# hbell99/DirectVoxGO

Measured on AMD Instinct MI355X. Metric: train rays/sec (8192-ray batch, 160^3 grid), higher is better.
Workload: dtype f32

## Files before the change

directvoxgo_amd/csrc/shade.hip:

```cpp
#include "common.h"
#include "x3.h"

#include <type_traits>


static int g_shade_experiment = 0;
static int g_shade_variant = 67;
extern "C" int dvgo_shade_wgrad_x3(const float* G1, const float* gz, const uint64_t* masks, const float* W3, const float* H1,
                                   const float* H2, const float* feat, int C, const float* emb, int E, const int64_t* ray_id,
                                   int64_t M, const int64_t* m_dev, int width, int diffuse, int n_parts, float* part, int form_b,
                                   void* stream);
extern "C" int dvgo_shade_bwd_x3(const float* g_rgb, const float* rgb, const uint64_t* masks, int64_t M, const int64_t* m_dev,
                                 const float* W1, const float* W2, const float* W3, int width, int d_in, int C, int diffuse,
                                 float* g_feat, float* G1, float* gz, void* scratch, int prebuilt, void* stream);

extern "C" int dvgo_shade_fwd_x3(const float* feat, int C, const float* emb, int E, const int64_t* ray_id, int64_t M, const int64_t* m_dev,
                                 const float* W1, const float* b1, const float* W2, const float* b2, const float* W3,
                                 const float* b3, int width, int d_in, int diffuse, float* rgb, float* H1, float* H2,
                                 uint64_t* masks, void* scratch, void* scratch_bwd, int experiment, void* stream);

#define SHADE_THREADS 768
#define SHADE_WAVES (SHADE_THREADS / 64)
#define SHADE_BWD_THREADS 1024
#define SHADE_BWD_WAVES (SHADE_BWD_THREADS / 64)

template <int WIDTH, int S1>
struct ShadeLds {
  static constexpr int T = WIDTH / 32;
  float w1a[T][S1][64];
  float w2a[T][T][16][64];
  float w3p[3][2][T * 16];
  float b1p[2][T * 16];
  float b2p[2][T * 16];
  float b3[4];
};

__device__ __forceinline__ int acc_feature(int t, int r, int h) { return 32 * t + (r & 3) + 8 * (r >> 2) + 4 * h; }

#define SHADE_STAGE_STRIDE 36
__device__ __forceinline__ void shade_store_tile(float* __restrict__ stage ,
                                                 const f32x16& acc, float* __restrict__ dst , int row_stride, int lane, int rows_valid) {
  const int smp = lane & 31, h = lane >> 5;
#pragma unroll
  for (int q = 0; q < 4; ++q)
    *reinterpret_cast<float4*>(stage + smp * SHADE_STAGE_STRIDE + 8 * q + 4 * h) =
        make_float4(acc[4 * q], acc[4 * q + 1], acc[4 * q + 2], acc[4 * q + 3]);
  const int c = lane & 7;
#pragma unroll
  for (int i = 0; i < 4; ++i) {
    const int r = (lane >> 3) + 8 * i;
    const float4 v = *reinterpret_cast<const float4*>(stage + r * SHADE_STAGE_STRIDE + 4 * c);
    if (r < rows_valid) *reinterpret_cast<float4*>(dst + (int64_t)r * row_stride + 4 * c) = v;
  }
}

template <int WIDTH, int S1>
__device__ __forceinline__ void shade_load_weights(ShadeLds<WIDTH, S1>& L, const float* __restrict__ W1,
                                                   const float* __restrict__ b1, const float* __restrict__ W2,
                                                   const float* __restrict__ b2, const float* __restrict__ W3,
                                                   const float* __restrict__ b3, int D_in) {
  constexpr int T = WIDTH / 32;
  const int tid = threadIdx.x, nt = blockDim.x;
  for (int i = tid; i < T * S1 * 64; i += nt) {
    const int l = i & 63, s = (i >> 6) % S1, t = (i >> 6) / S1;
    const int k = 2 * s + (l >> 5);
    (&L.w1a[0][0][0])[i] = (k < D_in) ? W1[(32 * t + (l & 31)) * D_in + k] : 0.0f;
  }
  for (int i = tid; i < T * T * 16 * 64; i += nt) {
    const int l = i & 63, r = (i >> 6) & 15, t = (i >> 10) % T, t2 = (i >> 10) / T;
    (&L.w2a[0][0][0][0])[i] = W2[(32 * t2 + (l & 31)) * WIDTH + acc_feature(t, r, l >> 5)];
  }
  for (int i = tid; i < 3 * 2 * T * 16; i += nt) {
    const int tr = i % (T * 16), h = (i / (T * 16)) & 1, c = i / (2 * T * 16);
    (&L.w3p[0][0][0])[i] = W3[c * WIDTH + acc_feature(tr >> 4, tr & 15, h)];
  }
  for (int i = tid; i < 2 * T * 16; i += nt) {
    const int tr = i % (T * 16), h = i / (T * 16);
    const int f = acc_feature(tr >> 4, tr & 15, h);
    (&L.b1p[0][0])[i] = b1[f];
    (&L.b2p[0][0])[i] = b2[f];
  }
  if (tid < 3) L.b3[tid] = b3[tid];
}

template <int WIDTH, int S1>
__device__ __forceinline__ void shade_tile_forward(const ShadeLds<WIDTH, S1>& L, const float (&x)[S1], int lane,
                                                   f32x16 (&acc1)[WIDTH / 32], float (&z)[3],
                                                   float* __restrict__ H2tile ,
                                                   float* __restrict__ stage, int rows_valid,
                                                   unsigned long long& mask2 ) {
  constexpr int T = WIDTH / 32;
  const int h = lane >> 5;
#pragma unroll
  for (int t = 0; t < T; ++t) {
#pragma unroll
    for (int r = 0; r < 16; ++r) acc1[t][r] = L.b1p[h][t * 16 + r];
#pragma unroll
    for (int s = 0; s < S1; ++s) acc1[t] = __builtin_amdgcn_mfma_f32_32x32x2f32(L.w1a[t][s][lane], x[s], acc1[t], 0, 0, 0);
#pragma unroll
    for (int r = 0; r < 16; ++r) acc1[t][r] = dvgo_relu(acc1[t][r]);
    __builtin_amdgcn_sched_barrier(0);
  }
  float p[3] = {0.0f, 0.0f, 0.0f};
  mask2 = 0ull;
#pragma unroll 1
  for (int t2 = 0; t2 < T; ++t2) {
    f32x16 acc2;
#pragma unroll
    for (int r = 0; r < 16; ++r) acc2[r] = L.b2p[h][t2 * 16 + r];
#pragma unroll
    for (int t = 0; t < T; ++t) {
#pragma unroll
      for (int r = 0; r < 16; ++r)
        acc2 = __builtin_amdgcn_mfma_f32_32x32x2f32(L.w2a[t2][t][r][lane], acc1[t][r], acc2, 0, 0, 0);
      __builtin_amdgcn_sched_barrier(0);
    }
#pragma unroll
    for (int r = 0; r < 16; ++r) acc2[r] = dvgo_relu(acc2[r]);
    if (H2tile != nullptr) {
      unsigned int bits = 0u;
#pragma unroll
      for (int r = 0; r < 16; ++r) bits |= dvgo_relu_bit(acc2[r]) << r;
      mask2 |= (unsigned long long)bits << (16 * t2);
      shade_store_tile(stage, acc2, H2tile + 32 * t2, WIDTH, lane, rows_valid);
    }
#pragma unroll
    for (int c = 0; c < 3; ++c) {
#pragma unroll
      for (int r = 0; r < 16; ++r) p[c] = fmaf(L.w3p[c][h][t2 * 16 + r], acc2[r], p[c]);
    }
  }
#pragma unroll
  for (int c = 0; c < 3; ++c) z[c] = p[c] + __shfl_xor(p[c], 32) + L.b3[c];
}

template <int S1>
__device__ __forceinline__ void shade_load_x(const float* __restrict__ feat, int C, int c_view0, int n_view,
                                             const float* __restrict__ emb, int E, int64_t row, int64_t ray,
                                             int lane, float (&x)[S1]) {
  const int h = lane >> 5;
  const float* fr = feat + row * C + c_view0;
  const float* er = emb + ray * E - n_view;
#pragma unroll
  for (int s = 0; s < S1; ++s) {
    const int k = 2 * s + h;
    float v = 0.0f;
    if (k < n_view) v = fr[k];
    else if (k < n_view + E) v = er[k];
    x[s] = v;
  }
}

template <int WIDTH, int S1, bool DIFFUSE>
__global__ void __launch_bounds__(SHADE_THREADS)
shade_fwd_kernel(const float* __restrict__ feat, int C, int c_view0, int n_view, const float* __restrict__ emb, int E,
                 const int64_t* __restrict__ ray_id, int64_t M_cap, const int64_t* __restrict__ m_dev, const float* __restrict__ W1,
                 const float* __restrict__ b1, const float* __restrict__ W2, const float* __restrict__ b2,
                 const float* __restrict__ W3, const float* __restrict__ b3, int D_in, float* __restrict__ rgb,
                 float* __restrict__ H1, float* __restrict__ H2, unsigned long long* __restrict__ masks, int experiment) {
  const int64_t M = m_dev ? (*m_dev < M_cap ? *m_dev : M_cap) : M_cap;
  constexpr int T = WIDTH / 32;
  __shared__ ShadeLds<WIDTH, S1> L;
  __shared__ __attribute__((aligned(16))) float s_stage[SHADE_WAVES][32 * SHADE_STAGE_STRIDE];
  shade_load_weights<WIDTH, S1>(L, W1, b1, W2, b2, W3, b3, D_in);
  __syncthreads();
  const int lane = threadIdx.x & 63, h = lane >> 5;
  float* stage = s_stage[threadIdx.x >> 6];
  const int64_t n_tiles = (M + 31) / 32;
  const int64_t gw = (int64_t)blockIdx.x * (blockDim.x >> 6) + (threadIdx.x >> 6);
  const int64_t nw = (int64_t)gridDim.x * (blockDim.x >> 6);
  for (int64_t tile = gw; tile < n_tiles; tile += nw) {
    const int64_t row = tile * 32 + (lane & 31);
    const bool valid = row < M;
    const int64_t rowc = valid ? row : (M - 1);
    float x[S1];
    if (experiment & 16) { for (int s = 0; s < S1; ++s) x[s] = 0.01f * (float)(lane + s); }
    else shade_load_x<S1>(feat, C, c_view0, n_view, emb, E, rowc, ray_id[rowc], lane, x);
    f32x16 acc1[T];
    float z[3];
    const int rows_valid = (int)(M - tile * 32 < 32 ? M - tile * 32 : 32);
    unsigned long long mask2;
    shade_tile_forward<WIDTH, S1>(L, x, lane, acc1, z, (H1 != nullptr && !(experiment & 32)) ? (H2 + tile * 32 * WIDTH) : nullptr,
                                  stage, rows_valid, mask2);
    if (valid) {
      if (h == 0) {
#pragma unroll
        for (int c = 0; c < 3; ++c) {
          const float zz = DIFFUSE ? z[c] + feat[row * C + c] : z[c];
          rgb[row * 3 + c] = 1.0f / (1.0f + expf(-zz));
        }
      }
      if (H1 != nullptr) {
        unsigned long long mask1 = 0ull;
#pragma unroll
        for (int t = 0; t < T; ++t) {
#pragma unroll
          for (int r = 0; r < 16; ++r) mask1 |= (unsigned long long)dvgo_relu_bit(acc1[t][r]) << (16 * t + r);
        }
        masks[(row * 2 + 0) * 2 + h] = mask1;
        masks[(row * 2 + 1) * 2 + h] = mask2;
      }
    }
    if (H1 != nullptr && !(experiment & 32)) {
#pragma unroll
      for (int t = 0; t < T; ++t) shade_store_tile(stage, acc1[t], H1 + tile * 32 * WIDTH + 32 * t, WIDTH, lane, rows_valid);
    }
  }
}

template <int WIDTH>
struct ShadeBwdLds {
  static constexpr int T = WIDTH / 32;
  float w2ta[T][T][16][64];
  float w1ta[T][16][64];
  float w3p[3][2][T * 16];
};

template <int WIDTH, bool DIFFUSE>
__global__ void __launch_bounds__(SHADE_BWD_THREADS)
shade_bwd_kernel(const float* __restrict__ g_rgb, const float* __restrict__ rgb,
                 const unsigned long long* __restrict__ masks, int64_t M_cap, const int64_t* __restrict__ m_dev,
                 const float* __restrict__ W1, const float* __restrict__ W2,
                 const float* __restrict__ W3, int D_in, int C, int c_view0, int n_view,
                 float* __restrict__ g_feat, float* __restrict__ G1, float* __restrict__ gz_out, int experiment) {
  const int64_t M = m_dev ? (*m_dev < M_cap ? *m_dev : M_cap) : M_cap;
  constexpr int T = WIDTH / 32;
  __shared__ ShadeBwdLds<WIDTH> L;
  __shared__ __attribute__((aligned(16))) float s_stage[SHADE_BWD_WAVES][32 * SHADE_STAGE_STRIDE];
  float* stage = s_stage[threadIdx.x >> 6];
  {
    const int tid = threadIdx.x, nt = blockDim.x;
    for (int i = tid; i < T * T * 16 * 64; i += nt) {
      const int l = i & 63, r = (i >> 6) & 15, t2 = (i >> 10) % T, tin = (i >> 10) / T;
      (&L.w2ta[0][0][0][0])[i] = W2[acc_feature(t2, r, l >> 5) * WIDTH + 32 * tin + (l & 31)];
    }
    for (int i = tid; i < T * 16 * 64; i += nt) {
      const int l = i & 63, r = (i >> 6) & 15, t = i >> 10;
      const int k = l & 31;
      (&L.w1ta[0][0][0])[i] = (k < D_in) ? W1[acc_feature(t, r, l >> 5) * D_in + k] : 0.0f;
    }
    for (int i = tid; i < 3 * 2 * T * 16; i += nt) {
      const int tr = i % (T * 16), h = (i / (T * 16)) & 1, c = i / (2 * T * 16);
      (&L.w3p[0][0][0])[i] = W3[c * WIDTH + acc_feature(tr >> 4, tr & 15, h)];
    }
  }
  __syncthreads();
  const int lane = threadIdx.x & 63, h = lane >> 5;
  const int64_t n_tiles = (M + 31) / 32;
  const int64_t gw = (int64_t)blockIdx.x * (blockDim.x >> 6) + (threadIdx.x >> 6);
  const int64_t nw = (int64_t)gridDim.x * (blockDim.x >> 6);
  for (int64_t tile = gw; tile < n_tiles; tile += nw) {
    const int64_t row = tile * 32 + (lane & 31);
    const bool valid = row < M;
    const int64_t rowc = valid ? row : (M - 1);
    float gz[3];
#pragma unroll
    for (int c = 0; c < 3; ++c) {
      const float o = rgb[rowc * 3 + c];
      gz[c] = valid ? g_rgb[rowc * 3 + c] * o * (1.0f - o) : 0.0f;
    }
    if (valid && h == 0) {
#pragma unroll
      for (int c = 0; c < 3; ++c) {
        gz_out[row * 3 + c] = gz[c];
        if (DIFFUSE) g_feat[row * C + c] = gz[c];
      }
    }
    const unsigned long long m1 = masks[(rowc * 2 + 0) * 2 + h];
    const unsigned long long m2 = masks[(rowc * 2 + 1) * 2 + h];
    f32x16 g2[T];
#pragma unroll
    for (int t2 = 0; t2 < T; ++t2) {
#pragma unroll
      for (int r = 0; r < 16; ++r) {
        const float v = fmaf(L.w3p[2][h][t2 * 16 + r], gz[2],
                             fmaf(L.w3p[1][h][t2 * 16 + r], gz[1], L.w3p[0][h][t2 * 16 + r] * gz[0]));
        g2[t2][r] = ((m2 >> (16 * t2 + r)) & 1ull) ? v : 0.0f;
      }
    }
    f32x16 gx;
#pragma unroll
    for (int r = 0; r < 16; ++r) gx[r] = 0.0f;
#pragma unroll 1
    for (int tin = 0; tin < T; ++tin) {
      f32x16 acc;
#pragma unroll
      for (int r = 0; r < 16; ++r) acc[r] = 0.0f;
#pragma unroll
      for (int t2 = 0; t2 < T; ++t2) {
#pragma unroll
        for (int r = 0; r < 16; ++r)
          acc = __builtin_amdgcn_mfma_f32_32x32x2f32(L.w2ta[tin][t2][r][lane], g2[t2][r], acc, 0, 0, 0);
        __builtin_amdgcn_sched_barrier(0);
      }
#pragma unroll
      for (int q = 0; q < 4; ++q) {
        const unsigned int mb = (unsigned int)(m1 >> (16 * tin + 4 * q)) & 15u;
        acc[4 * q + 0] = (mb & 1u) ? acc[4 * q + 0] : 0.0f;
        acc[4 * q + 1] = (mb & 2u) ? acc[4 * q + 1] : 0.0f;
        acc[4 * q + 2] = (mb & 4u) ? acc[4 * q + 2] : 0.0f;
        acc[4 * q + 3] = (mb & 8u) ? acc[4 * q + 3] : 0.0f;
      }
      if (!(experiment & 1))
        shade_store_tile(stage, acc, G1 + tile * 32 * WIDTH + 32 * tin, WIDTH, lane,
                         (int)(M - tile * 32 < 32 ? M - tile * 32 : 32));
#pragma unroll
      for (int r = 0; r < 16; ++r)
        gx = __builtin_amdgcn_mfma_f32_32x32x2f32(L.w1ta[tin][r][lane], acc[r], gx, 0, 0, 0);
    }
    if (valid) {
#pragma unroll
      for (int r = 0; r < 16; ++r) {
        const int k = (r & 3) + 8 * (r >> 2) + 4 * h;
        if (k < n_view) g_feat[row * C + c_view0 + k] = gx[r];
      }
    }
  }
}

template <int WIDTH>
struct ShadeWgradLds {
  float g1[1][32][WIDTH], h1[1][32][WIDTH], h2[1][32][WIDTH];
  float x[1][32][40];
  float gz[1][32][4];
  unsigned int m2[1][32][2][2];
};

typedef const __attribute__((address_space(1))) void* dvgo_gptr_t;
typedef __attribute__((address_space(3))) void* dvgo_lptr_t;

template <int WIDTH>
__global__ void __launch_bounds__(2 * WIDTH) __attribute__((amdgpu_num_vgpr(104)))
shade_wgrad_kernel(const float* __restrict__ G1, const float* __restrict__ gz, const unsigned int* __restrict__ masks,
                   const float* __restrict__ W3, const float* __restrict__ H1, const float* __restrict__ H2, const float* __restrict__ feat, int C,
                   int c_view0, int n_view, const float* __restrict__ emb, int E, const int64_t* __restrict__ ray_id,
                   int64_t M_cap, const int64_t* __restrict__ m_dev,
                   float* __restrict__ part ) {
  const int64_t M = m_dev ? (*m_dev < M_cap ? *m_dev : M_cap) : M_cap;
  constexpr int T = WIDTH / 32;
  static_assert(T == 4 || T == 2, "widths 128 and 64");
  constexpr int TPR = 2 * T;
  constexpr int NXI = 40 / TPR;
  constexpr int LPR = WIDTH / 4;
  constexpr int RPI = 64 / LPR;
  __shared__ __attribute__((aligned(16))) ShadeWgradLds<WIDTH> L;
  const int tid = threadIdx.x, lane = tid & 63, h = lane >> 5, j = lane & 31, w = tid >> 6;
  f32x16 aW2[T], aW1;
  float vW3[3] = {0.0f, 0.0f, 0.0f};
  float vW1[8];
#pragma unroll
  for (int t = 0; t < T; ++t)
#pragma unroll
    for (int r = 0; r < 16; ++r) aW2[t][r] = 0.0f;
#pragma unroll
  for (int r = 0; r < 16; ++r) aW1[r] = 0.0f;
#pragma unroll
  for (int kk = 0; kk < 8; ++kk) vW1[kk] = 0.0f;
  float sb1 = 0.0f, sb2 = 0.0f, gz_acc = 0.0f;
  const float w30 = W3[32 * w + j], w31 = W3[WIDTH + 32 * w + j], w32 = W3[2 * WIDTH + 32 * w + j];
  const int m_half = (j >> 2) & 1, m_word = w >> 1, m_bit = 16 * (w & 1) + (j & 3) + 4 * (j >> 3);
  const int d_in = n_view + E;
  const int64_t n_tiles = (M + 31) / 32;

  float px[NXI], pgz;
  unsigned int pm2;
  bool pvalid, pgvalid;
  int64_t ray_nx;
  const int xrow = tid / TPR, xcol = tid - xrow * TPR;
  {
    const int64_t row = (int64_t)blockIdx.x * 32 + xrow;
    ray_nx = M > 0 ? ray_id[row < M ? row : M - 1] : 0;
  }
#define SHADE_WGRAD_DMA(TILE, BUF)                                                                              \
  {                                                                                                             \
    const int64_t r0_ = (TILE) * 32;                                                                            \
    {                                                                                                           \
      const int64_t row = r0_ + xrow;                                                                           \
      const int64_t rc = row < M ? row : M - 1;                                                                 \
      const float* fr = feat + rc * C + c_view0;                                                                \
      const float* er = emb + ray_nx * E - n_view;                     \
      _Pragma("unroll") for (int i = 0; i < NXI; ++i) {                          \
        const int k = xcol + TPR * i;                                                                           \
        const int kc = k < d_in ? k : d_in - 1;                                                                 \
        px[i] = *((kc < n_view) ? fr + kc : er + kc);                                                           \
      }                                                                                                         \
      pvalid = row < M;                                                                                         \
      const int64_t row2 = r0_ + (int64_t)gridDim.x * 32 + xrow;                                                \
      ray_nx = ray_id[row2 < M ? row2 : M - 1];                        \
    }                                                                                                           \
    {                                                                                                           \
      const int64_t row = r0_ + ((tid & 127) >> 2);                                                             \
      const int64_t rc = row < M ? row : M - 1;                                                                 \
      pgz = gz[rc * 3 + ((tid & 3) < 3 ? (tid & 3) : 0)];                                                       \
      pgvalid = (tid & 3) < 3 && row < M;                                                                       \
       \
      pm2 = masks[rc * 8 + 4 + (tid & 3)];                                                                      \
    }                                                                                                           \
                           \
    _Pragma("unroll") for (int i = 0; i < 4; ++i) {             \
      const int rl = (4 * w + i) * RPI;                  \
      const int64_t row = r0_ + rl + lane / LPR;                                                                \
      const int64_t off = (row < M ? row : M - 1) * WIDTH + 4 * (lane % LPR);                                   \
      __builtin_amdgcn_global_load_lds((dvgo_gptr_t)(G1 + off), (dvgo_lptr_t)&L.g1[BUF][rl][0], 16, 0, 0);     \
      __builtin_amdgcn_global_load_lds((dvgo_gptr_t)(H1 + off), (dvgo_lptr_t)&L.h1[BUF][rl][0], 16, 0, 0);     \
      __builtin_amdgcn_global_load_lds((dvgo_gptr_t)(H2 + off), (dvgo_lptr_t)&L.h2[BUF][rl][0], 16, 0, 0);     \
    }                                                                                                           \
  }

  constexpr int buf = 0;
  for (int64_t tile = blockIdx.x; tile < n_tiles; tile += gridDim.x) {
    SHADE_WGRAD_DMA(tile, 0);
    asm volatile("" : "+v"(px[0]), "+v"(px[1]), "+v"(px[2]), "+v"(px[3]), "+v"(px[4]), "+v"(pgz), "+v"(pm2));
    if (NXI > 5) asm volatile("" : "+v"(px[NXI - 5]), "+v"(px[NXI - 4]), "+v"(px[NXI - 3]), "+v"(px[NXI - 2]), "+v"(px[NXI - 1]));
#pragma unroll
    for (int i = 0; i < NXI; ++i) L.x[buf][xrow][xcol + TPR * i] = (pvalid && xcol + TPR * i < d_in) ? px[i] : 0.0f;
    if (tid < 128) {
      gz_acc += pgvalid ? pgz : 0.0f;
      L.gz[buf][tid >> 2][tid & 3] = pgvalid ? pgz : 0.0f;
      (&L.m2[buf][tid >> 2][0][0])[tid & 3] = pm2;
    }
    __builtin_amdgcn_s_waitcnt(0x0F70);
    __syncthreads();
    const int rows_valid = (int)(M - tile * 32 < 32 ? M - tile * 32 : 32);
#pragma unroll 4
    for (int s = 0; s < 16; ++s) {
      const int row = 2 * s + h;
      const float4 gzr = *reinterpret_cast<const float4*>(&L.gz[buf][row][0]);
      const float g2v = fmaf(w32, gzr.z, fmaf(w31, gzr.y, w30 * gzr.x));
      const float a2 = ((L.m2[buf][row][m_half][m_word] >> m_bit) & 1u) ? g2v : 0.0f;
      const float a1 = row < rows_valid ? L.g1[buf][row][32 * w + j] : 0.0f;
      sb2 += a2; sb1 += a1;
#pragma unroll
      for (int t = 0; t < T; ++t)
        aW2[t] = __builtin_amdgcn_mfma_f32_32x32x2f32(a2, L.h1[buf][row][32 * t + j], aW2[t], 0, 0, 0);
      aW1 = __builtin_amdgcn_mfma_f32_32x32x2f32(a1, L.x[buf][row][j], aW1, 0, 0, 0);
      const float4 xa = *reinterpret_cast<const float4*>(&L.x[buf][row][32]);
      const float4 xb = *reinterpret_cast<const float4*>(&L.x[buf][row][36]);
      vW1[0] = fmaf(a1, xa.x, vW1[0]); vW1[1] = fmaf(a1, xa.y, vW1[1]); vW1[2] = fmaf(a1, xa.z, vW1[2]);
      vW1[3] = fmaf(a1, xa.w, vW1[3]); vW1[4] = fmaf(a1, xb.x, vW1[4]); vW1[5] = fmaf(a1, xb.y, vW1[5]);
      vW1[6] = fmaf(a1, xb.z, vW1[6]); vW1[7] = fmaf(a1, xb.w, vW1[7]);
      const float hv = L.h2[buf][row][32 * w + j];
      vW3[0] = fmaf(gzr.x, hv, vW3[0]); vW3[1] = fmaf(gzr.y, hv, vW3[1]); vW3[2] = fmaf(gzr.z, hv, vW3[2]);
    }
    __syncthreads();
  }
#undef SHADE_WGRAD_DMA
  float* p = part + (int64_t)blockIdx.x * (WIDTH * WIDTH + WIDTH * 64 + 32 * WIDTH + 3 * WIDTH);
  float* pW2 = p;
  float* pW1 = pW2 + WIDTH * WIDTH;
  float* pW3 = pW1 + WIDTH * 64;
  float* pb = pW3 + 32 * WIDTH;
#pragma unroll
  for (int r = 0; r < 16; ++r) {
    const int i = (r & 3) + 8 * (r >> 2) + 4 * h;
#pragma unroll
    for (int t = 0; t < T; ++t) pW2[(32 * w + i) * WIDTH + 32 * t + j] = aW2[t][r];
    pW1[(32 * w + i) * 64 + j] = aW1[r];
  }
#pragma unroll
  for (int kk = 0; kk < 8; ++kk) {
    const float v = vW1[kk] + __shfl_xor(vW1[kk], 32);
    if (h == 0) pW1[(32 * w + j) * 64 + 32 + kk] = v;
  }
  if (h == 0) {
#pragma unroll
    for (int kk = 8; kk < 32; ++kk) pW1[(32 * w + j) * 64 + 32 + kk] = 0.0f;
  }
#pragma unroll
  for (int c = 0; c < 3; ++c) {
    const float v = vW3[c] + __shfl_xor(vW3[c], 32);
    if (h == 0) pW3[c * WIDTH + 32 * w + j] = v;
  }
  float gz_sum = gz_acc;
  gz_sum += __shfl_xor(gz_sum, 4); gz_sum += __shfl_xor(gz_sum, 8);
  gz_sum += __shfl_xor(gz_sum, 16); gz_sum += __shfl_xor(gz_sum, 32);
  sb1 += __shfl_xor(sb1, 32); sb2 += __shfl_xor(sb2, 32);
  if (h == 0) {
    pb[32 * w + j] = sb1;
    pb[WIDTH + 32 * w + j] = sb2;
    if (j < 8) pb[2 * WIDTH + 8 * w + j] = (w < 2 && j < 3) ? gz_sum : 0.0f;
    if (T == 2 && j >= 16) pb[2 * WIDTH + 16 * w + j] = 0.0f;
  }
}

__device__ __forceinline__ unsigned lds_addr(const void* p) {
  return (unsigned)(uintptr_t)(const __attribute__((address_space(3))) void*)p;
}
template <int OFF> __device__ __forceinline__ float lds_f32(unsigned a) {
  float v; asm volatile("ds_read_b32 %0, %1 offset:%2" : "=v"(v) : "v"(a), "n"(OFF)); return v;
}
template <int OFF> __device__ __forceinline__ unsigned lds_u32(unsigned a) {
  unsigned v; asm volatile("ds_read_b32 %0, %1 offset:%2" : "=v"(v) : "v"(a), "n"(OFF)); return v;
}
typedef float dvgo_f32x4 __attribute__((ext_vector_type(4)));
template <int OFF> __device__ __forceinline__ dvgo_f32x4 lds_f32x4(unsigned a) {
  dvgo_f32x4 v; asm volatile("ds_read_b128 %0, %1 offset:%2" : "=v"(v) : "v"(a), "n"(OFF)); return v;
}
template <int I, int N, typename F> __device__ __forceinline__ void static_for(F&& f) {
  if constexpr (I < N) { f(std::integral_constant<int, I>{}); static_for<I + 1, N>(f); }
}

template <int WIDTH>
struct ShadeWgradRing {
  static constexpr int NB = 2, NR = 4, TR = 16;
  float g1[NB][TR][WIDTH], h1[NB][TR][WIDTH], h2[NB][TR][WIDTH];
  float xf[NB][TR][16];
  float xe[NB][TR][32];
  float gz[NB][TR][4];
  unsigned int m2[NB][TR][4];
  unsigned int rid[NR][64];
};

template <int T>
struct WgradOperands {
  dvgo_f32x4 gq, xa, xb;
  unsigned mw;
  float g1v, h1v[T], xv, h2v;
};

#define DVGO_OOB 0x80000000u

template <int WIDTH>
__global__ void __launch_bounds__(2 * WIDTH, 2)
shade_wgrad_ring_kernel(const float* __restrict__ G1, const float* __restrict__ gz, const unsigned int* __restrict__ masks,
                        const float* __restrict__ W3, const float* __restrict__ H1, const float* __restrict__ H2,
                        const float* __restrict__ feat, int C, int c_view0, int n_view, const float* __restrict__ emb, int E,
                        const int64_t* __restrict__ ray_id, int64_t M_cap, const int64_t* __restrict__ m_dev,
                        float* __restrict__ part ,
                        float* __restrict__ total, int total_size ) {
#if defined(__HIP_DEVICE_COMPILE__)
  for (int i = blockIdx.x * blockDim.x + threadIdx.x; i < total_size; i += gridDim.x * blockDim.x) total[i] = 0.0f;
  int64_t M;
  {
    const int64_t m = m_dev ? (*m_dev < M_cap ? *m_dev : M_cap) : M_cap;
    M = ((int64_t)__builtin_amdgcn_readfirstlane((int)(m >> 32)) << 32) | (unsigned)__builtin_amdgcn_readfirstlane((int)m);
  }
  using Ring = ShadeWgradRing<WIDTH>;
  constexpr int T = WIDTH / 32, NW = T, NB = Ring::NB, NR = Ring::NR, TR = Ring::TR;
  static_assert(T == 4 || T == 2, "widths 128 and 64");
  constexpr int LPR = WIDTH / 4;
  constexpr int RPI = 64 / LPR;
  constexpr int IPW = TR / RPI / NW;
  constexpr int FPW = 4 / NW, EPW = 8 / NW;
  static_assert(IPW == 2 && NB == 2, "double buffer: the wait at the top of a tile is vmcnt(0)");
  __shared__ __attribute__((aligned(16))) Ring L;
  const int tid = threadIdx.x, lane = tid & 63, h = lane >> 5, j = lane & 31;
  const int w = __builtin_amdgcn_readfirstlane(tid >> 6);
  f32x16 aW2[T], aW1;
  float vW3[3] = {0.0f, 0.0f, 0.0f}, vW1[8], sgz[3] = {0.0f, 0.0f, 0.0f};
#pragma unroll
  for (int t = 0; t < T; ++t)
#pragma unroll
    for (int r = 0; r < 16; ++r) aW2[t][r] = 0.0f;
#pragma unroll
  for (int r = 0; r < 16; ++r) aW1[r] = 0.0f;
#pragma unroll
  for (int kk = 0; kk < 8; ++kk) vW1[kk] = 0.0f;
  float sb1 = 0.0f, sb2 = 0.0f;
  const float w30 = W3[32 * w + j], w31 = W3[WIDTH + 32 * w + j], w32 = W3[2 * WIDTH + 32 * w + j];
  const int m_idx = 2 * ((j >> 2) & 1) + (w >> 1), m_bit = 16 * (w & 1) + (j & 3) + 4 * (j >> 3);
  const int d_in = n_view + E;
  const int n_tiles = (int)((M + TR - 1) / TR);
  auto tile_of = [&](int k) { return (int)blockIdx.x + k * (int)gridDim.x; };

  const unsigned rows_b = (unsigned)(M * WIDTH * 4);
  const auto bG1 = __builtin_amdgcn_make_buffer_rsrc((void*)G1, 0, rows_b, 0x00020000);
  const auto bH1 = __builtin_amdgcn_make_buffer_rsrc((void*)H1, 0, rows_b, 0x00020000);
  const auto bH2 = __builtin_amdgcn_make_buffer_rsrc((void*)H2, 0, rows_b, 0x00020000);
  const auto bF = __builtin_amdgcn_make_buffer_rsrc((void*)feat, 0, (unsigned)(M * C * 4), 0x00020000);
  const auto bE = __builtin_amdgcn_make_buffer_rsrc((void*)emb, 0, DVGO_OOB, 0x00020000);
  const auto bGz = __builtin_amdgcn_make_buffer_rsrc((void*)gz, 0, (unsigned)(M * 12), 0x00020000);
  const auto bM = __builtin_amdgcn_make_buffer_rsrc((void*)masks, 0, (unsigned)(M * 32), 0x00020000);
  const auto bR = __builtin_amdgcn_make_buffer_rsrc((void*)ray_id, 0, (unsigned)(M * 8), 0x00020000);
  unsigned vo_bulk[IPW], vo_f[FPW], vo_ecol[EPW];
  int e_row[EPW];
#pragma unroll
  for (int i = 0; i < IPW; ++i) vo_bulk[i] = (unsigned)(((IPW * w + i) * RPI + lane / LPR) * WIDTH * 4 + 16 * (lane % LPR));
#pragma unroll
  for (int i = 0; i < FPW; ++i) {
    const int e = 64 * (w + NW * i) + lane, row = e >> 4, col = e & 15;
    vo_f[i] = col < n_view ? (unsigned)((row * C + c_view0 + col) * 4) : DVGO_OOB;
  }
#pragma unroll
  for (int i = 0; i < EPW; ++i) {
    const int e = 64 * (w + NW * i) + lane, col = e & 31;
    e_row[i] = e >> 5;
    vo_ecol[i] = col < E ? (unsigned)(col * 4) : DVGO_OOB;
  }
  const unsigned vo_gz = (lane & 3) < 3 ? (unsigned)(((lane >> 2) * 3 + (lane & 3)) * 4) : DVGO_OOB;
  const unsigned vo_m2 = (unsigned)(((lane >> 2) * 8 + 4 + (lane & 3)) * 4);
  const unsigned vo_rid = (unsigned)((lane & (TR - 1)) * 8);

  auto issue = [&](int t) {
    const int sl = t & (NB - 1);
    const unsigned r0 = (unsigned)__builtin_amdgcn_readfirstlane(tile_of(t) * TR);
#pragma unroll
    for (int i = 0; i < IPW; ++i) {
      const int rl = (IPW * w + i) * RPI;
      __builtin_amdgcn_raw_ptr_buffer_load_lds(bG1, (dvgo_lptr_t)&L.g1[sl][rl][0], 16, vo_bulk[i], r0 * (WIDTH * 4), 0, 0);
      __builtin_amdgcn_raw_ptr_buffer_load_lds(bH1, (dvgo_lptr_t)&L.h1[sl][rl][0], 16, vo_bulk[i], r0 * (WIDTH * 4), 0, 0);
      __builtin_amdgcn_raw_ptr_buffer_load_lds(bH2, (dvgo_lptr_t)&L.h2[sl][rl][0], 16, vo_bulk[i], r0 * (WIDTH * 4), 0, 0);
    }
#pragma unroll
    for (int i = 0; i < FPW; ++i)
      __builtin_amdgcn_raw_ptr_buffer_load_lds(bF, (dvgo_lptr_t)(&L.xf[sl][0][0] + 64 * (w + NW * i)), 4, vo_f[i], r0 * (unsigned)(C * 4), 0, 0);
    unsigned rids[EPW];
#pragma unroll
    for (int i = 0; i < EPW; ++i) rids[i] = lds_u32<0>(lds_addr(&L.rid[t & (NR - 1)][e_row[i]]));
    if constexpr (EPW == 2) asm volatile("s_waitcnt lgkmcnt(0)" : "+v"(rids[0]), "+v"(rids[1]));
    else asm volatile("s_waitcnt lgkmcnt(0)" : "+v"(rids[0]), "+v"(rids[1]), "+v"(rids[EPW - 2]), "+v"(rids[EPW - 1]));
#pragma unroll
    for (int i = 0; i < EPW; ++i)
      __builtin_amdgcn_raw_ptr_buffer_load_lds(bE, (dvgo_lptr_t)(&L.xe[sl][0][0] + 64 * (w + NW * i)), 4,
                                               vo_ecol[i] + rids[i] * (unsigned)(E * 4), 0, 0, 0);
    const unsigned rn = (unsigned)__builtin_amdgcn_readfirstlane(tile_of(t + 2) * TR);
    const int rsl = (t + 2) & (NR - 1);
    auto small = [&](int which) {
      if (which == 0) __builtin_amdgcn_raw_ptr_buffer_load_lds(bGz, (dvgo_lptr_t)&L.gz[sl][0][0], 4, vo_gz, r0 * 12u, 0, 0);
      else if (which == 1) __builtin_amdgcn_raw_ptr_buffer_load_lds(bM, (dvgo_lptr_t)&L.m2[sl][0][0], 4, vo_m2, r0 * 32u, 0, 0);
      else __builtin_amdgcn_raw_ptr_buffer_load_lds(bR, (dvgo_lptr_t)&L.rid[rsl][0], 4, vo_rid, rn * 8u, 0, 0);
    };
    if constexpr (NW == 4) {
      small(w < 2 ? w : 2);
    } else {
      small(w);
      small(2);
    }
  };

  const unsigned a_gz = lds_addr(&L.gz[0][h][0]), a_mw = lds_addr(&L.m2[0][h][m_idx]);
  const unsigned a_g1 = lds_addr(&L.g1[0][h][32 * w + j]), a_h1 = lds_addr(&L.h1[0][h][j]);
  const unsigned a_h2 = lds_addr(&L.h2[0][h][32 * w + j]);
  const bool x_in_f = j < n_view;
  const unsigned a_x = x_in_f ? lds_addr(&L.xf[0][h][j]) : lds_addr(&L.xe[0][h][j - n_view]);
  const unsigned x_slot = x_in_f ? (unsigned)(TR * 16 * 4) : (unsigned)(TR * 32 * 4), x_step = x_in_f ? 128u : 256u;
  const bool trail = d_in > 32;
  const unsigned a_xa = lds_addr(&L.xe[0][h][trail ? 32 - n_view : 0]);
  constexpr unsigned SLOT_ROWS = TR * WIDTH * 4;
  using Ops = WgradOperands<T>;
  auto wait_ops = [&](Ops& o) {
    if constexpr (T == 4)
      asm volatile("s_waitcnt lgkmcnt(0)" : "+v"(o.gq), "+v"(o.xa), "+v"(o.xb), "+v"(o.mw), "+v"(o.g1v), "+v"(o.h1v[0]),
                   "+v"(o.h1v[1]), "+v"(o.h1v[2]), "+v"(o.h1v[3]), "+v"(o.xv), "+v"(o.h2v));
    else
      asm volatile("s_waitcnt lgkmcnt(0)" : "+v"(o.gq), "+v"(o.xa), "+v"(o.xb), "+v"(o.mw), "+v"(o.g1v), "+v"(o.h1v[0]),
                   "+v"(o.h1v[1]), "+v"(o.xv), "+v"(o.h2v));
  };

  if (tid < 64) {
#pragma unroll
    for (int t = 0; t < 2; ++t) {
      const int64_t row = (int64_t)tile_of(t) * TR + (tid & (TR - 1));
      L.rid[t][tid] = row < M ? (unsigned int)ray_id[row] : 0u;
    }
  }
  __syncthreads();
#pragma unroll
  for (int t = 0; t < NB - 1; ++t) issue(t);
  for (int k = 0; tile_of(k) < n_tiles; ++k) {
    const int sl = k & (NB - 1);
    asm volatile("s_waitcnt vmcnt(0)\n\ts_waitcnt lgkmcnt(0)\n\ts_barrier" ::: "memory");
    issue(k + NB - 1);
    const unsigned b_gz = a_gz + sl * (TR * 16), b_mw = a_mw + sl * (TR * 16), b_g1 = a_g1 + sl * SLOT_ROWS;
    const unsigned b_h1 = a_h1 + sl * SLOT_ROWS, b_h2 = a_h2 + sl * SLOT_ROWS;
    const unsigned b_xa = a_xa + sl * (TR * 32 * 4);
    unsigned b_x = a_x + sl * x_slot;
    Ops ops[2];
    float a2s[2], a1s[2];
    auto read_ops = [&](auto Sc, Ops& o) {
      constexpr int s = decltype(Sc)::value;
      o.gq = lds_f32x4<32 * s>(b_gz);
      o.mw = lds_u32<32 * s>(b_mw);
      o.g1v = lds_f32<8 * WIDTH * s>(b_g1);
      static_for<0, T>([&](auto Tc) { constexpr int t = decltype(Tc)::value; o.h1v[t] = lds_f32<8 * WIDTH * s + 128 * t>(b_h1); });
      o.xv = lds_f32<0>(b_x);
      b_x += x_step;
      o.xa = lds_f32x4<256 * s>(b_xa);
      o.xb = lds_f32x4<256 * s + 16>(b_xa);
      o.h2v = lds_f32<8 * WIDTH * s>(b_h2);
    };
    auto prep = [&](const Ops& o, float& a2, float& a1) {
      const float g2v = fmaf(w32, o.gq.z, fmaf(w31, o.gq.y, w30 * o.gq.x));
      a2 = ((o.mw >> m_bit) & 1u) ? g2v : 0.0f;
      a1 = o.g1v;
    };
    read_ops(std::integral_constant<int, 0>{}, ops[0]);
    wait_ops(ops[0]);
    prep(ops[0], a2s[0], a1s[0]);
    static_for<0, TR / 2>([&](auto Sc) {
      constexpr int s = decltype(Sc)::value;
      constexpr bool more = s + 1 < TR / 2;
      Ops& cur = ops[s & 1];
      Ops& nxt = ops[(s + 1) & 1];
      const float a2 = a2s[s & 1], a1 = a1s[s & 1];
      aW2[0] = __builtin_amdgcn_mfma_f32_32x32x2f32(a2, cur.h1v[0], aW2[0], 0, 0, 0);
      if constexpr (more) read_ops(std::integral_constant<int, s + 1>{}, nxt);
      sb2 += a2; sb1 += a1;
      sgz[0] += cur.gq.x; sgz[1] += cur.gq.y; sgz[2] += cur.gq.z;
      __builtin_amdgcn_sched_barrier(0);
      aW2[1] = __builtin_amdgcn_mfma_f32_32x32x2f32(a2, cur.h1v[1], aW2[1], 0, 0, 0);
      vW1[0] = fmaf(a1, cur.xa.x, vW1[0]); vW1[1] = fmaf(a1, cur.xa.y, vW1[1]); vW1[2] = fmaf(a1, cur.xa.z, vW1[2]);
      vW1[3] = fmaf(a1, cur.xa.w, vW1[3]);
      vW3[0] = fmaf(cur.gq.x, cur.h2v, vW3[0]); vW3[1] = fmaf(cur.gq.y, cur.h2v, vW3[1]); vW3[2] = fmaf(cur.gq.z, cur.h2v, vW3[2]);
      __builtin_amdgcn_sched_barrier(0);
      if constexpr (T == 4) aW2[2] = __builtin_amdgcn_mfma_f32_32x32x2f32(a2, cur.h1v[2], aW2[2], 0, 0, 0);
      vW1[4] = fmaf(a1, cur.xb.x, vW1[4]); vW1[5] = fmaf(a1, cur.xb.y, vW1[5]); vW1[6] = fmaf(a1, cur.xb.z, vW1[6]);
      vW1[7] = fmaf(a1, cur.xb.w, vW1[7]);
      if constexpr (more) wait_ops(nxt);
      __builtin_amdgcn_sched_barrier(0);
      if constexpr (T == 4) aW2[3] = __builtin_amdgcn_mfma_f32_32x32x2f32(a2, cur.h1v[3], aW2[3], 0, 0, 0);
      if constexpr (more) prep(nxt, a2s[(s + 1) & 1], a1s[(s + 1) & 1]);
      __builtin_amdgcn_sched_barrier(0);
      aW1 = __builtin_amdgcn_mfma_f32_32x32x2f32(a1, cur.xv, aW1, 0, 0, 0);
      __builtin_amdgcn_sched_barrier(0);
    });
  }
  asm volatile("s_waitcnt vmcnt(0)" ::: "memory");
  float* p = part + (int64_t)blockIdx.x * (WIDTH * WIDTH + WIDTH * 64 + 32 * WIDTH + 3 * WIDTH);
  float* pW2 = p;
  float* pW1 = pW2 + WIDTH * WIDTH;
  float* pW3 = pW1 + WIDTH * 64;
  float* pb = pW3 + 32 * WIDTH;
#pragma unroll
  for (int r = 0; r < 16; ++r) {
    const int i = (r & 3) + 8 * (r >> 2) + 4 * h;
#pragma unroll
    for (int t = 0; t < T; ++t) pW2[(32 * w + i) * WIDTH + 32 * t + j] = aW2[t][r];
    pW1[(32 * w + i) * 64 + j] = aW1[r];
  }
#pragma unroll
  for (int kk = 0; kk < 8; ++kk) {
    const float v = vW1[kk] + __shfl_xor(vW1[kk], 32);
    if (h == 0) pW1[(32 * w + j) * 64 + 32 + kk] = (trail && 32 + kk < d_in) ? v : 0.0f;
  }
  if (h == 0) {
#pragma unroll
    for (int kk = 8; kk < 32; ++kk) pW1[(32 * w + j) * 64 + 32 + kk] = 0.0f;
  }
#pragma unroll
  for (int c = 0; c < 3; ++c) {
    const float v = vW3[c] + __shfl_xor(vW3[c], 32);
    if (h == 0) pW3[c * WIDTH + 32 * w + j] = v;
    sgz[c] += __shfl_xor(sgz[c], 32);
  }
  sb1 += __shfl_xor(sb1, 32); sb2 += __shfl_xor(sb2, 32);
  if (h == 0) {
    pb[32 * w + j] = sb1;
    pb[WIDTH + 32 * w + j] = sb2;
    if (j < 8) pb[2 * WIDTH + 8 * w + j] = (w == 0 && j < 3) ? sgz[j] : 0.0f;
    if (T == 2 && j >= 16) pb[2 * WIDTH + 16 * w + j] = 0.0f;
  }
#endif
}
typedef float dvgo_f32x2 __attribute__((ext_vector_type(2)));
template <int O0, int O1> __device__ __forceinline__ dvgo_f32x2 lds_f32_pair_st64(unsigned a) {
  dvgo_f32x2 v; asm volatile("ds_read2st64_b32 %0, %1 offset0:%2 offset1:%3" : "=v"(v) : "v"(a), "n"(O0), "n"(O1)); return v;
}
template <int O0, int O1> __device__ __forceinline__ dvgo_f32x2 lds_f32_pair(unsigned a) {
  dvgo_f32x2 v; asm volatile("ds_read2_b32 %0, %1 offset0:%2 offset1:%3" : "=v"(v) : "v"(a), "n"(O0), "n"(O1)); return v;
}
template <int OFF> __device__ __forceinline__ u32x4 lds_u32x4(unsigned a) {
  u32x4 v; asm volatile("ds_read_b128 %0, %1 offset:%2" : "=v"(v) : "v"(a), "n"(OFF)); return v;
}
template <int OFF> __device__ __forceinline__ void lds_store_u32x4(unsigned a, u32x4 v) {
  asm volatile("ds_write_b128 %0, %1 offset:%2" :: "v"(a), "v"(v), "n"(OFF) : "memory");
}

template <int WIDTH>
struct ShadeWgradRingX3 : ShadeWgradRing<WIDTH> {
  u32x4 fb[WIDTH / 32 + 2][3][64];
};

template <int WIDTH>
__global__ void __launch_bounds__(2 * WIDTH, 2)
shade_wgrad_ring_x3_kernel(const float* __restrict__ G1, const float* __restrict__ gz, const unsigned int* __restrict__ masks,
                           const float* __restrict__ W3, const float* __restrict__ H1, const float* __restrict__ H2,
                           const float* __restrict__ feat, int C, int c_view0, int n_view, const float* __restrict__ emb, int E,
                           const int64_t* __restrict__ ray_id, int64_t M_cap, const int64_t* __restrict__ m_dev,
                           float* __restrict__ part, float* __restrict__ total, int total_size) {
#if defined(__HIP_DEVICE_COMPILE__)
  for (int i = blockIdx.x * blockDim.x + threadIdx.x; i < total_size; i += gridDim.x * blockDim.x) total[i] = 0.0f;
  int64_t M;
  {
    const int64_t m = m_dev ? (*m_dev < M_cap ? *m_dev : M_cap) : M_cap;
    M = ((int64_t)__builtin_amdgcn_readfirstlane((int)(m >> 32)) << 32) | (unsigned)__builtin_amdgcn_readfirstlane((int)m);
  }
  using Ring = ShadeWgradRingX3<WIDTH>;
  constexpr int T = WIDTH / 32, NW = T, NB = Ring::NB, NR = Ring::NR, TR = Ring::TR;
  static_assert(T == 4 || T == 2, "widths 128 and 64");
  constexpr int LPR = WIDTH / 4, RPI = 64 / LPR, IPW = TR / RPI / NW;
  constexpr int DW = NW == 4 ? 2 : NW, FPW = 4 / DW, EPW = 8 / DW;
  static_assert(IPW == 2 && NB == 2 && TR == 16, "double buffer of 16-row tiles: the wait at the top of a tile is vmcnt(0)");
  __shared__ __attribute__((aligned(16))) Ring L;
  const int tid = threadIdx.x, lane = tid & 63, h = lane >> 5, j = lane & 31;
  const int w = __builtin_amdgcn_readfirstlane(tid >> 6);
  const int dw = NW == 4 ? w - 2 : w;
  f32x16 aW2[T], aW1[2];
  float vW3[3] = {0.0f, 0.0f, 0.0f}, sgz[3] = {0.0f, 0.0f, 0.0f};
#pragma unroll
  for (int t = 0; t < T; ++t)
#pragma unroll
    for (int r = 0; r < 16; ++r) aW2[t][r] = 0.0f;
#pragma unroll
  for (int q = 0; q < 2; ++q)
#pragma unroll
    for (int r = 0; r < 16; ++r) aW1[q][r] = 0.0f;
  float sb1 = 0.0f, sb2 = 0.0f;
  const float w30 = W3[32 * w + j], w31 = W3[WIDTH + 32 * w + j], w32 = W3[2 * WIDTH + 32 * w + j];
  const int m_idx = 2 * ((j >> 2) & 1) + (w >> 1);
  const unsigned m_bit = 16 * (w & 1) + (j & 3) + 4 * (j >> 3);
  const int d_in = n_view + E;
  const int n_tiles = (int)((M + TR - 1) / TR);
  auto tile_of = [&](int k) { return (int)blockIdx.x + k * (int)gridDim.x; };
  const unsigned rows_b = (unsigned)(M * WIDTH * 4);
  const auto bG1 = __builtin_amdgcn_make_buffer_rsrc((void*)G1, 0, rows_b, 0x00020000);
  const auto bH1 = __builtin_amdgcn_make_buffer_rsrc((void*)H1, 0, rows_b, 0x00020000);
  const auto bH2 = __builtin_amdgcn_make_buffer_rsrc((void*)H2, 0, rows_b, 0x00020000);
  const auto bF = __builtin_amdgcn_make_buffer_rsrc((void*)feat, 0, (unsigned)(M * C * 4), 0x00020000);
  const auto bE = __builtin_amdgcn_make_buffer_rsrc((void*)emb, 0, DVGO_OOB, 0x00020000);
  const auto bGz = __builtin_amdgcn_make_buffer_rsrc((void*)gz, 0, (unsigned)(M * 12), 0x00020000);
  const auto bM = __builtin_amdgcn_make_buffer_rsrc((void*)masks, 0, (unsigned)(M * 32), 0x00020000);
  const auto bR = __builtin_amdgcn_make_buffer_rsrc((void*)ray_id, 0, (unsigned)(M * 8), 0x00020000);
  unsigned vo_bulk[IPW], vo_f[FPW], vo_ecol[EPW];
  int e_row[EPW];
#pragma unroll
  for (int i = 0; i < IPW; ++i) vo_bulk[i] = (unsigned)(((IPW * w + i) * RPI + lane / LPR) * WIDTH * 4 + 16 * (lane % LPR));
#pragma unroll
  for (int i = 0; i < FPW; ++i) {
    const int e = 64 * ((dw < 0 ? 0 : dw) + DW * i) + lane, row = e >> 4, col = e & 15;
    vo_f[i] = col < n_view ? (unsigned)((row * C + c_view0 + col) * 4) : DVGO_OOB;
  }
#pragma unroll
  for (int i = 0; i < EPW; ++i) {
    const int e = 64 * ((dw < 0 ? 0 : dw) + DW * i) + lane, col = e & 31;
    e_row[i] = e >> 5;
    vo_ecol[i] = col < E ? (unsigned)(col * 4) : DVGO_OOB;
  }
  const unsigned vo_gz = (lane & 3) < 3 ? (unsigned)(((lane >> 2) * 3 + (lane & 3)) * 4) : DVGO_OOB;
  const unsigned vo_m2 = (unsigned)(((lane >> 2) * 8 + 4 + (lane & 3)) * 4);
  const unsigned vo_rid = (unsigned)((lane & (TR - 1)) * 8);
  auto issue = [&](int t) {
    const int sl = t & (NB - 1);
    const unsigned r0 = (unsigned)__builtin_amdgcn_readfirstlane(tile_of(t) * TR);
#pragma unroll
    for (int i = 0; i < IPW; ++i) {
      const int rl = (IPW * w + i) * RPI;
      __builtin_amdgcn_raw_ptr_buffer_load_lds(bG1, (dvgo_lptr_t)&L.g1[sl][rl][0], 16, vo_bulk[i], r0 * (WIDTH * 4), 0, 0);
      __builtin_amdgcn_raw_ptr_buffer_load_lds(bH1, (dvgo_lptr_t)&L.h1[sl][rl][0], 16, vo_bulk[i], r0 * (WIDTH * 4), 0, 0);
      __builtin_amdgcn_raw_ptr_buffer_load_lds(bH2, (dvgo_lptr_t)&L.h2[sl][rl][0], 16, vo_bulk[i], r0 * (WIDTH * 4), 0, 0);
    }
    if (dw < 0) return;
#pragma unroll
    for (int i = 0; i < FPW; ++i)
      __builtin_amdgcn_raw_ptr_buffer_load_lds(bF, (dvgo_lptr_t)(&L.xf[sl][0][0] + 64 * (dw + DW * i)), 4, vo_f[i], r0 * (unsigned)(C * 4), 0, 0);
    unsigned rids[EPW];
#pragma unroll
    for (int i = 0; i < EPW; ++i) rids[i] = lds_u32<0>(lds_addr(&L.rid[t & (NR - 1)][e_row[i]]));
    asm volatile("s_waitcnt lgkmcnt(0)" : "+v"(rids[0]), "+v"(rids[1]), "+v"(rids[2]), "+v"(rids[3]));
#pragma unroll
    for (int i = 0; i < EPW; ++i)
      __builtin_amdgcn_raw_ptr_buffer_load_lds(bE, (dvgo_lptr_t)(&L.xe[sl][0][0] + 64 * (dw + DW * i)), 4,
                                               vo_ecol[i] + rids[i] * (unsigned)(E * 4), 0, 0, 0);
    const unsigned rn = (unsigned)__builtin_amdgcn_readfirstlane(tile_of(t + 2) * TR);
    const int rsl = (t + 2) & (NR - 1);
    auto small = [&](int which) {
      if (which == 0) __builtin_amdgcn_raw_ptr_buffer_load_lds(bGz, (dvgo_lptr_t)&L.gz[sl][0][0], 4, vo_gz, r0 * 12u, 0, 0);
      else if (which == 1) __builtin_amdgcn_raw_ptr_buffer_load_lds(bM, (dvgo_lptr_t)&L.m2[sl][0][0], 4, vo_m2, r0 * 32u, 0, 0);
      else __builtin_amdgcn_raw_ptr_buffer_load_lds(bR, (dvgo_lptr_t)&L.rid[rsl][0], 4, vo_rid, rn * 8u, 0, 0);
    };
    if (dw == 0) { small(0); small(1); } else small(2);
  };
  const unsigned a_gz = lds_addr(&L.gz[0][8 * h][0]), a_mw = lds_addr(&L.m2[0][8 * h][m_idx]);
  const unsigned a_g1 = lds_addr(&L.g1[0][8 * h][32 * w + j]), a_h1 = lds_addr(&L.h1[0][8 * h][32 * w + j]);
  const unsigned a_h2 = lds_addr(&L.h2[0][8 * h][32 * w + j]);
  const int xcol = 32 * (w & 1) + j;
  const bool x_in_f = xcol < n_view, x_ok = xcol < d_in;
  const unsigned a_x = x_in_f ? lds_addr(&L.xf[0][8 * h][xcol]) : lds_addr(&L.xe[0][8 * h][x_ok ? xcol - n_view : 0]);
  const unsigned a_fb = lds_addr(&L.fb[0][0][lane]);
  constexpr unsigned SLOT_ROWS = TR * WIDTH * 4, FB_TILE = 3 * 64 * 16, FB_PIECE = 64 * 16;
  if (tid < 64) {
#pragma unroll
    for (int t = 0; t < 2; ++t) {
      const int64_t row = (int64_t)tile_of(t) * TR + (tid & (TR - 1));
      L.rid[t][tid] = row < M ? (unsigned int)ray_id[row] : 0u;
    }
  }
  __syncthreads();
#pragma unroll
  for (int t = 0; t < NB - 1; ++t) issue(t);
  for (int k = 0; tile_of(k) < n_tiles; ++k) {
    const int sl = k & (NB - 1);
    asm volatile("s_waitcnt vmcnt(0)\n\ts_waitcnt lgkmcnt(0)\n\ts_barrier" ::: "memory");
    issue(k + NB - 1);
    const unsigned b_gz = a_gz + sl * (TR * 16), b_mw = a_mw + sl * (TR * 16), b_g1 = a_g1 + sl * SLOT_ROWS;
    const unsigned b_h1 = a_h1 + sl * SLOT_ROWS, b_h2 = a_h2 + sl * SLOT_ROWS;
    const unsigned b_x = a_x + sl * (x_in_f ? (unsigned)(TR * 16 * 4) : (unsigned)(TR * 32 * 4));
    dvgo_f32x4 gq[8];
    unsigned mw[8];
    float g1v[8], h1v[8], h2v[8], xv[8];
    constexpr int RS = WIDTH * 4 / 256;
    static_for<0, 4>([&](auto Ec) {
      constexpr int e = 2 * decltype(Ec)::value;
      const dvgo_f32x2 v = lds_f32_pair_st64<e * RS, (e + 1) * RS>(b_h1);
      h1v[e] = v.x; h1v[e + 1] = v.y;
    });
    if (w < 2) {
      if (x_in_f) static_for<0, 8>([&](auto Ec) { constexpr int e = decltype(Ec)::value; xv[e] = lds_f32<e * 16 * 4>(b_x); });
      else static_for<0, 8>([&](auto Ec) { constexpr int e = decltype(Ec)::value; xv[e] = lds_f32<e * 32 * 4>(b_x); });
    }
    static_for<0, 8>([&](auto Ec) {
      constexpr int e = decltype(Ec)::value;
      gq[e] = lds_f32x4<16 * e>(b_gz);
    });
    static_for<0, 4>([&](auto Ec) {
      constexpr int e = 2 * decltype(Ec)::value;
      const dvgo_f32x2 m = lds_f32_pair<4 * e, 4 * (e + 1)>(b_mw);
      mw[e] = __float_as_uint(m.x); mw[e + 1] = __float_as_uint(m.y);
      const dvgo_f32x2 a = lds_f32_pair_st64<e * RS, (e + 1) * RS>(b_g1);
      g1v[e] = a.x; g1v[e + 1] = a.y;
      const dvgo_f32x2 b = lds_f32_pair_st64<e * RS, (e + 1) * RS>(b_h2);
      h2v[e] = b.x; h2v[e + 1] = b.y;
    });
    asm volatile("s_waitcnt lgkmcnt(0)" : "+v"(h1v[0]), "+v"(h1v[1]), "+v"(h1v[2]), "+v"(h1v[3]), "+v"(h1v[4]), "+v"(h1v[5]),
                 "+v"(h1v[6]), "+v"(h1v[7]), "+v"(gq[0]), "+v"(gq[1]), "+v"(gq[2]), "+v"(gq[3]), "+v"(gq[4]), "+v"(gq[5]), "+v"(gq[6]),
                 "+v"(gq[7]));
    asm volatile("" : "+v"(mw[0]), "+v"(mw[1]), "+v"(mw[2]), "+v"(mw[3]), "+v"(mw[4]), "+v"(mw[5]), "+v"(mw[6]), "+v"(mw[7]),
                 "+v"(g1v[0]), "+v"(g1v[1]), "+v"(g1v[2]), "+v"(g1v[3]), "+v"(g1v[4]), "+v"(g1v[5]), "+v"(g1v[6]), "+v"(g1v[7]));
    asm volatile("" : "+v"(h2v[0]), "+v"(h2v[1]), "+v"(h2v[2]), "+v"(h2v[3]), "+v"(h2v[4]), "+v"(h2v[5]), "+v"(h2v[6]), "+v"(h2v[7]));
    {
      u32x4 p0, p1, p2;
      x3_split8(h1v, p0, p1, p2);
      lds_store_u32x4<0>(a_fb + w * FB_TILE, p0);
      lds_store_u32x4<FB_PIECE>(a_fb + w * FB_TILE, p1);
      lds_store_u32x4<2 * FB_PIECE>(a_fb + w * FB_TILE, p2);
      if (w < 2) {
        asm volatile("" : "+v"(xv[0]), "+v"(xv[1]), "+v"(xv[2]), "+v"(xv[3]), "+v"(xv[4]), "+v"(xv[5]), "+v"(xv[6]), "+v"(xv[7]));
#pragma unroll
        for (int e = 0; e < 8; ++e) xv[e] = x_ok ? xv[e] : 0.0f;
        x3_split8(xv, p0, p1, p2);
        lds_store_u32x4<0>(a_fb + (T + w) * FB_TILE, p0);
        lds_store_u32x4<FB_PIECE>(a_fb + (T + w) * FB_TILE, p1);
        lds_store_u32x4<2 * FB_PIECE>(a_fb + (T + w) * FB_TILE, p2);
      }
    }
    u32x4 a2f[3], a1f[3];
    {
      float a2[8];
#pragma unroll
      for (int e = 0; e < 8; ++e) {
        const float g2v = fmaf(w32, gq[e].z, fmaf(w31, gq[e].y, w30 * gq[e].x));
        a2[e] = __uint_as_float(__float_as_uint(g2v) & (unsigned)__builtin_amdgcn_sbfe((int)mw[e], m_bit, 1u));
        sb2 += a2[e]; sb1 += g1v[e];
        vW3[0] = fmaf(gq[e].x, h2v[e], vW3[0]); vW3[1] = fmaf(gq[e].y, h2v[e], vW3[1]); vW3[2] = fmaf(gq[e].z, h2v[e], vW3[2]);
      }
      if (w == 0) {
#pragma unroll
        for (int e = 0; e < 8; ++e) { sgz[0] += gq[e].x; sgz[1] += gq[e].y; sgz[2] += gq[e].z; }
      }
      x3_split8(a2, a2f[0], a2f[1], a2f[2]);
      x3_split8(g1v, a1f[0], a1f[1], a1f[2]);
    }
    asm volatile("s_waitcnt lgkmcnt(0)\n\ts_barrier" ::: "memory");
    u32x4 fr[2][2][3];
    auto read_pair = [&](auto Pc, u32x4 (&f)[2][3]) {
      constexpr int p = decltype(Pc)::value;
#pragma unroll
      for (int q = 0; q < 3; ++q) {
        f[0][q] = lds_u32x4<(2 * p) * FB_TILE>(a_fb + q * FB_PIECE);
        f[1][q] = lds_u32x4<(2 * p + 1) * FB_TILE>(a_fb + q * FB_PIECE);
      }
    };
    auto wait_pair = [&](u32x4 (&f)[2][3]) {
      asm volatile("s_waitcnt lgkmcnt(0)" : "+v"(f[0][0]), "+v"(f[0][1]), "+v"(f[0][2]), "+v"(f[1][0]), "+v"(f[1][1]), "+v"(f[1][2]));
    };
    auto mfma_pair = [&](f32x16& accA, f32x16& accB, const u32x4 (&a)[3], const u32x4 (&f)[2][3]) {
#define X3D_MF(ACC, A, B) ACC = __builtin_amdgcn_mfma_f32_32x32x16_bf16(__builtin_bit_cast(bf16x8, A), __builtin_bit_cast(bf16x8, B), ACC, 0, 0, 0)
      X3D_MF(accA, a[2], f[0][0]); X3D_MF(accB, a[2], f[1][0]);
      X3D_MF(accA, a[1], f[0][1]); X3D_MF(accB, a[1], f[1][1]);
      X3D_MF(accA, a[0], f[0][2]); X3D_MF(accB, a[0], f[1][2]);
      X3D_MF(accA, a[1], f[0][0]); X3D_MF(accB, a[1], f[1][0]);
      X3D_MF(accA, a[0], f[0][1]); X3D_MF(accB, a[0], f[1][1]);
      X3D_MF(accA, a[0], f[0][0]); X3D_MF(accB, a[0], f[1][0]);
#undef X3D_MF
    };
    constexpr int NP = T / 2 + 1;
    read_pair(std::integral_constant<int, 0>{}, fr[0]);
    static_for<0, NP>([&](auto Pc) {
      constexpr int p = decltype(Pc)::value;
      wait_pair(fr[p & 1]);
      if constexpr (p + 1 < NP) read_pair(std::integral_constant<int, p + 1>{}, fr[(p + 1) & 1]);
      if constexpr (p < T / 2) mfma_pair(aW2[2 * p], aW2[2 * p + 1], a2f, fr[p & 1]);
      else mfma_pair(aW1[0], aW1[1], a1f, fr[p & 1]);
      __builtin_amdgcn_sched_barrier(0);
    });
  }
  asm volatile("s_waitcnt vmcnt(0)" ::: "memory");
  float* p = part + (int64_t)blockIdx.x * (WIDTH * WIDTH + WIDTH * 64 + 32 * WIDTH + 3 * WIDTH);
  float* pW2 = p;
  float* pW1 = pW2 + WIDTH * WIDTH;
  float* pW3 = pW1 + WIDTH * 64;
  float* pb = pW3 + 32 * WIDTH;
#pragma unroll
  for (int r = 0; r < 16; ++r) {
    const int i = (r & 3) + 8 * (r >> 2) + 4 * h;
#pragma unroll
    for (int t = 0; t < T; ++t) pW2[(32 * w + i) * WIDTH + 32 * t + j] = aW2[t][r];
    pW1[(32 * w + i) * 64 + j] = aW1[0][r];
    pW1[(32 * w + i) * 64 + 32 + j] = aW1[1][r];
  }
#pragma unroll
  for (int c = 0; c < 3; ++c) {
    const float v = vW3[c] + __shfl_xor(vW3[c], 32);
    if (h == 0) pW3[c * WIDTH + 32 * w + j] = v;
    sgz[c] += __shfl_xor(sgz[c], 32);
  }
  sb1 += __shfl_xor(sb1, 32); sb2 += __shfl_xor(sb2, 32);
  if (h == 0) {
    pb[32 * w + j] = sb1;
    pb[WIDTH + 32 * w + j] = sb2;
    if (j < 8) pb[2 * WIDTH + 8 * w + j] = (w == 0 && j < 3) ? sgz[j] : 0.0f;
    if (T == 2 && j >= 16) pb[2 * WIDTH + 16 * w + j] = 0.0f;
  }
#endif
}
#undef DVGO_OOB

#define SHADE_REDUCE_SLICES 16
__global__ void __launch_bounds__(256)
shade_wgrad_reduce_kernel(const float* __restrict__ part, int n_parts, int n, int W, int d_in, float* __restrict__ out) {
  const int i = blockIdx.x * blockDim.x + threadIdx.x;
  if (i >= n) return;
  int o;
  const int nW2 = W * W, nW1 = W * 64, nW3 = 32 * W;
  if (i < nW2) o = i;
  else if (i < nW2 + nW1) {
    const int r = (i - nW2) >> 6, c = (i - nW2) & 63;
    o = c < d_in ? nW2 + r * d_in + c : -1;
  } else if (i < nW2 + nW1 + nW3) {
    const int e = i - nW2 - nW1;
    o = e < 3 * W ? nW2 + W * d_in + e : -1;
  } else {
    const int e = i - nW2 - nW1 - nW3, base = nW2 + W * d_in + 3 * W;
    if (e < 2 * W) o = base + e;
    else {
      const int c = e - 2 * W;
      o = c < 3 ? base + 2 * W + c : (c >= 8 && c < 11) ? base + 2 * W + c - 8 : -1;
    }
  }
  if (o < 0) return;
  const int per = (n_parts + SHADE_REDUCE_SLICES - 1) / SHADE_REDUCE_SLICES;
  const int p0 = blockIdx.y * per, p1 = min(n_parts, p0 + per);
  float a0 = 0.0f, a1 = 0.0f, a2 = 0.0f, a3 = 0.0f;
  int p = p0;
  for (; p + 4 <= p1; p += 4) {
    a0 += part[(int64_t)p * n + i];
    a1 += part[(int64_t)(p + 1) * n + i];
    a2 += part[(int64_t)(p + 2) * n + i];
    a3 += part[(int64_t)(p + 3) * n + i];
  }
  for (; p < p1; ++p) a0 += part[(int64_t)p * n + i];
  if (p1 > p0) atomicAdd(out + o, (a0 + a1) + (a2 + a3));
}

extern "C" {

int dvgo_shade_fwd(const float* feat, int C, const float* emb, int E, const int64_t* ray_id, int64_t M, const int64_t* m_dev,
                   const float* W1, const float* b1, const float* W2, const float* b2, const float* W3,
                   const float* b3, int width, int d_in, int diffuse, float* rgb, float* H1, float* H2,
                   uint64_t* masks, void* scratch, void* scratch_bwd, void* stream) {
  if (M < 0 || C <= 0 || E < 0) return DVGO_EINVAL;
  if (M == 0) return 0;
  if (!feat || !emb || !ray_id || !W1 || !b1 || !W2 || !b2 || !W3 || !b3 || !rgb) return DVGO_EINVAL;
  if ((H1 == nullptr) != (H2 == nullptr) || (H1 == nullptr) != (masks == nullptr)) return DVGO_EINVAL;
  const int c_view0 = diffuse ? 3 : 0;
  const int n_view = C - c_view0;
  if (n_view < 0 || d_in != n_view + E) return DVGO_EINVAL;
  if ((width != 128 && width != 64) || d_in > 40) return DVGO_ERANGE;
  if ((g_shade_variant & 1) && scratch != nullptr)
    return dvgo_shade_fwd_x3(feat, C, emb, E, ray_id, M, m_dev, W1, b1, W2, b2, W3, b3, width, d_in, diffuse, rgb, H1, H2, masks,
                             scratch, (g_shade_variant & 2) ? scratch_bwd : nullptr, g_shade_experiment, stream);
  hipStream_t s = (hipStream_t)stream;
  const int64_t n_tiles = (M + 31) / 32;
  const int64_t cap = width == 128 ? 256 : 512;
  int blocks = (int)((n_tiles + SHADE_WAVES - 1) / SHADE_WAVES < cap ? (n_tiles + SHADE_WAVES - 1) / SHADE_WAVES : cap);
#define DVGO_SHADE(W, S1, DIFF)                                                                           \
  shade_fwd_kernel<W, S1, DIFF><<<blocks, SHADE_THREADS, 0, s>>>(feat, C, c_view0, n_view, emb, E, ray_id, M, m_dev, W1, b1, W2, \
                                                          b2, W3, b3, d_in, rgb, H1, H2, (unsigned long long*)masks, g_shade_experiment)
  if (width == 128) {
    if (d_in <= 36) { if (diffuse) DVGO_SHADE(128, 18, true); else DVGO_SHADE(128, 18, false); }
    else            { if (diffuse) DVGO_SHADE(128, 20, true); else DVGO_SHADE(128, 20, false); }
  } else {
    if (d_in <= 12) { if (diffuse) DVGO_SHADE(64, 6, true); else DVGO_SHADE(64, 6, false); }
    else            { if (diffuse) DVGO_SHADE(64, 20, true); else DVGO_SHADE(64, 20, false); }
  }
#undef DVGO_SHADE
  DVGO_LAUNCH_CHECK();
  return 0;
}

int dvgo_shade_experiment(int flags) { g_shade_experiment = flags; return 0; }

int dvgo_shade_variant(int flags) { const int old = g_shade_variant; if (flags >= 0) g_shade_variant = flags; return old; }

int dvgo_shade_bwd(const float* g_rgb, const float* rgb, const uint64_t* masks, int64_t M, const int64_t* m_dev,
                   const float* W1, const float* W2, const float* W3, int width, int d_in, int C, int diffuse,
                   float* g_feat, float* G1, float* gz, void* scratch, int prebuilt, void* stream) {
  if (M < 0 || C <= 0) return DVGO_EINVAL;
  if (M == 0) return 0;
  if (!g_rgb || !rgb || !masks || !W1 || !W2 || !W3 || !g_feat || !G1 || !gz) return DVGO_EINVAL;
  const int c_view0 = diffuse ? 3 : 0;
  const int n_view = C - c_view0;
  if ((width != 128 && width != 64) || n_view < 0 || n_view > 32 || d_in < n_view) return DVGO_ERANGE;
  if ((g_shade_variant & 2) && scratch != nullptr)
    return dvgo_shade_bwd_x3(g_rgb, rgb, masks, M, m_dev, W1, W2, W3, width, d_in, C, diffuse, g_feat, G1, gz, scratch, prebuilt, stream);
  hipStream_t s = (hipStream_t)stream;
  const int64_t n_tiles = (M + 31) / 32;
  const int64_t cap = width == 128 ? 256 : 512;
  int blocks = (int)((n_tiles + SHADE_BWD_WAVES - 1) / SHADE_BWD_WAVES < cap ? (n_tiles + SHADE_BWD_WAVES - 1) / SHADE_BWD_WAVES : cap);
#define DVGO_SHADE_BWD(W, DIFF)                                                                                                       \
  shade_bwd_kernel<W, DIFF><<<blocks, SHADE_BWD_THREADS, 0, s>>>(g_rgb, rgb, (const unsigned long long*)masks, M, m_dev, W1, W2, W3, d_in, C, c_view0, \
                                                            n_view, g_feat, G1, gz, g_shade_experiment)
  if (width == 128) { if (diffuse) DVGO_SHADE_BWD(128, true); else DVGO_SHADE_BWD(128, false); }
  else              { if (diffuse) DVGO_SHADE_BWD(64, true); else DVGO_SHADE_BWD(64, false); }
#undef DVGO_SHADE_BWD
  DVGO_LAUNCH_CHECK();
  return 0;
}

int dvgo_shade_wgrad(const float* G1, const float* gz, const uint64_t* masks, const float* W3, const float* H1,
                     const float* H2, const float* feat, int C, const float* emb, int E, const int64_t* ray_id, int64_t M,
                     const int64_t* m_dev, int width, int diffuse, int n_parts, float* part, float* total, void* stream) {
  if (M < 0 || n_parts <= 0 || C <= 0 || E < 0) return DVGO_EINVAL;
  if (!G1 || !gz || !masks || !W3 || !H1 || !H2 || !feat || !emb || !ray_id || !part || !total) return DVGO_EINVAL;
  const int c_view0 = diffuse ? 3 : 0;
  const int n_view = C - c_view0;
  if ((width != 128 && width != 64) || n_view < 0 || n_view + E > 40) return DVGO_ERANGE;
  bool ring = false;
  if (g_shade_variant & (4 | 32)) {
    const int form_b = (g_shade_variant & 32) ? 2 : (g_shade_variant & 16) ? 1 : 0;
    if (!form_b && n_parts > 256) n_parts = 256;
    const int rc = dvgo_shade_wgrad_x3(G1, gz, masks, W3, H1, H2, feat, C, emb, E, ray_id, M, m_dev, width, diffuse, n_parts, part,
                                       form_b, stream);
    if (rc != 0) return rc;
  } else if (!(g_shade_variant & 8) && n_view <= 16 && E <= 32 && (n_view + E <= 32 || (n_view % 4 == 0 && n_view >= 8)) &&
             M * width * 4 < ((int64_t)1 << 31) && M * C * 4 < ((int64_t)1 << 31)) {
    if (n_parts > 512) n_parts = 512;
    ring = true;
    const int tsz = width * width + width * (n_view + E) + 5 * width + 3;
    if ((g_shade_variant & 64) && width == 128)
      shade_wgrad_ring_x3_kernel<128><<<n_parts, 256, 0, (hipStream_t)stream>>>(
          G1, gz, (const unsigned int*)masks, W3, H1, H2, feat, C, c_view0, n_view, emb, E, ray_id, M, m_dev, part, total, tsz);
    else if (g_shade_variant & 64)
      shade_wgrad_ring_x3_kernel<64><<<n_parts, 128, 0, (hipStream_t)stream>>>(
          G1, gz, (const unsigned int*)masks, W3, H1, H2, feat, C, c_view0, n_view, emb, E, ray_id, M, m_dev, part, total, tsz);
    else if (width == 128)
      shade_wgrad_ring_kernel<128><<<n_parts, 256, 0, (hipStream_t)stream>>>(
          G1, gz, (const unsigned int*)masks, W3, H1, H2, feat, C, c_view0, n_view, emb, E, ray_id, M, m_dev, part, total, tsz);
    else
      shade_wgrad_ring_kernel<64><<<n_parts, 128, 0, (hipStream_t)stream>>>(
          G1, gz, (const unsigned int*)masks, W3, H1, H2, feat, C, c_view0, n_view, emb, E, ray_id, M, m_dev, part, total, tsz);
  } else if (width == 128)
    shade_wgrad_kernel<128><<<n_parts, 256, 0, (hipStream_t)stream>>>(
        G1, gz, (const unsigned int*)masks, W3, H1, H2, feat, C, c_view0, n_view, emb, E, ray_id, M, m_dev, part);
  else
    shade_wgrad_kernel<64><<<n_parts, 128, 0, (hipStream_t)stream>>>(
        G1, gz, (const unsigned int*)masks, W3, H1, H2, feat, C, c_view0, n_view, emb, E, ray_id, M, m_dev, part);
  DVGO_LAUNCH_CHECK();
  const int psize = width * width + width * 64 + 32 * width + 3 * width;
  const int d_in = n_view + E;
  const int tsize = width * width + width * d_in + 3 * width + 2 * width + 3;
  if (!ring && hipMemsetAsync(total, 0, (size_t)tsize * sizeof(float), (hipStream_t)stream) != hipSuccess) return DVGO_EINVAL;
  shade_wgrad_reduce_kernel<<<dim3((psize + 255) / 256, SHADE_REDUCE_SLICES), 256, 0, (hipStream_t)stream>>>(part, n_parts, psize,
                                                                                                       width, d_in, total);
  DVGO_LAUNCH_CHECK();
  return 0;
}

}
```

directvoxgo_amd/csrc/shade_x3.hip:

```cpp
#include "common.h"
#include "x3.h"

#ifndef X3_THREADS
#define X3_THREADS 512
#endif
#define X3_WAVES (X3_THREADS / 64)
#ifndef X3_BWD_THREADS
#define X3_BWD_THREADS 512
#endif
#define X3_BWD_WAVES (X3_BWD_THREADS / 64)
#define X3_STAGE_ROWS 16
#define X3_STAGE_STRIDE 36

__device__ __forceinline__ int x3_acc_feature(int t, int r, int h) { return 32 * t + (r & 3) + 8 * (r >> 2) + 4 * h; }

__device__ __forceinline__ void x3_split1(float v, unsigned short& s0, unsigned short& s1, unsigned short& s2) {
  const unsigned int h = x3_pack(v, 0.f) & 0xffffu;
  const float r = v - __uint_as_float(h << 16);
  const unsigned int m = x3_pack(r, 0.f) & 0xffffu;
  const float q = r - __uint_as_float(m << 16);
  s0 = (unsigned short)h; s1 = (unsigned short)m; s2 = (unsigned short)(x3_pack(q, 0.f) & 0xffffu);
}

template <int WIDTH, int KS1>
struct X3Img {
  static constexpr int T = WIDTH / 32;
  u32x4 w1s[T][KS1][3][64];
  u32x4 w2s[T][2 * T][3][64];
  float w3p[3][2][T * 16];
  float b1p[2][T * 16];
  float b2p[2][T * 16];
  float b3[4];
};

template <int WIDTH, int KS1>
struct X3Lds : X3Img<WIDTH, KS1> {
  float stage[X3_WAVES][X3_STAGE_ROWS * X3_STAGE_STRIDE];
};

template <typename Img>
__device__ __forceinline__ void x3_copy_image(Img* __restrict__ dst , const void* __restrict__ src) {
  static_assert(sizeof(Img) % 16 == 0, "16-byte pieces");
  const u32x4* g = reinterpret_cast<const u32x4*>(src);
  u32x4* l = reinterpret_cast<u32x4*>(dst);
  for (int i = threadIdx.x; i < (int)(sizeof(Img) / 16); i += blockDim.x) l[i] = g[i];
}

__device__ __forceinline__ void x3_store_tile(float* __restrict__ stage, const f32x16& acc, float* __restrict__ dst, int row_stride,
                                              int lane, int rows_valid) {
  const int smp = lane & 31, h = lane >> 5;
#pragma unroll
  for (int half = 0; half < 2; ++half) {
    if ((smp >> 4) == half) {
#pragma unroll
      for (int q = 0; q < 4; ++q)
        *reinterpret_cast<float4*>(stage + (smp & 15) * X3_STAGE_STRIDE + 8 * q + 4 * h) =
            make_float4(acc[4 * q], acc[4 * q + 1], acc[4 * q + 2], acc[4 * q + 3]);
    }
    const int c = lane & 7;
#pragma unroll
    for (int i = 0; i < 2; ++i) {
      const int rl = (lane >> 3) + 8 * i;
      const float4 v = *reinterpret_cast<const float4*>(stage + rl * X3_STAGE_STRIDE + 4 * c);
      const int r = 16 * half + rl;
      if (r < rows_valid) *reinterpret_cast<float4*>(dst + (int64_t)r * row_stride + 4 * c) = v;
    }
  }
}

template <int WIDTH, int KS1>
__device__ __forceinline__ void
x3_prep_fwd_body(X3Img<WIDTH, KS1>* __restrict__ Lp, const float* __restrict__ W1, const float* __restrict__ b1,
                 const float* __restrict__ W2, const float* __restrict__ b2, const float* __restrict__ W3,
                 const float* __restrict__ b3, int D_in, const int tid, const int nt) {
  constexpr int T = WIDTH / 32;
  X3Img<WIDTH, KS1>& L = *Lp;
  for (int i = tid; i < T * KS1 * 64 * 8; i += nt) {
    const int j = i & 7, l = (i >> 3) & 63, s = (i >> 9) % KS1, t = (i >> 9) / KS1;
    const int k = 16 * s + 8 * (l >> 5) + j;
    const float v = (k < D_in) ? W1[(32 * t + (l & 31)) * D_in + k] : 0.0f;
    unsigned short p0, p1, p2;
    x3_split1(v, p0, p1, p2);
    reinterpret_cast<unsigned short*>(&L.w1s[t][s][0][l])[j] = p0;
    reinterpret_cast<unsigned short*>(&L.w1s[t][s][1][l])[j] = p1;
    reinterpret_cast<unsigned short*>(&L.w1s[t][s][2][l])[j] = p2;
  }
  for (int i = tid; i < T * 2 * T * 64 * 8; i += nt) {
    const int j = i & 7, l = (i >> 3) & 63, ks = (i >> 9) % (2 * T), t2 = (i >> 9) / (2 * T);
    const int k = 16 * ks + 8 * (j >> 2) + 4 * (l >> 5) + (j & 3);
    const float v = W2[(32 * t2 + (l & 31)) * WIDTH + k];
    unsigned short p0, p1, p2;
    x3_split1(v, p0, p1, p2);
    reinterpret_cast<unsigned short*>(&L.w2s[t2][ks][0][l])[j] = p0;
    reinterpret_cast<unsigned short*>(&L.w2s[t2][ks][1][l])[j] = p1;
    reinterpret_cast<unsigned short*>(&L.w2s[t2][ks][2][l])[j] = p2;
  }
  for (int i = tid; i < 3 * 2 * T * 16; i += nt) {
    const int tr = i % (T * 16), h = (i / (T * 16)) & 1, c = i / (2 * T * 16);
    (&L.w3p[0][0][0])[i] = W3[c * WIDTH + x3_acc_feature(tr >> 4, tr & 15, h)];
  }
  for (int i = tid; i < 2 * T * 16; i += nt) {
    const int tr = i % (T * 16), h = i / (T * 16);
    const int f = x3_acc_feature(tr >> 4, tr & 15, h);
    (&L.b1p[0][0])[i] = b1[f];
    (&L.b2p[0][0])[i] = b2[f];
  }
  if (tid < 4) L.b3[tid] = tid < 3 ? b3[tid] : 0.0f;
}

template <int WIDTH, int KS1, bool DIFFUSE>
__global__ void __launch_bounds__(X3_THREADS)
shade_fwd_x3_kernel(const float* __restrict__ feat, int C, int c_view0, int n_view, const float* __restrict__ emb, int E,
                    const int64_t* __restrict__ ray_id, int64_t M_cap, const int64_t* __restrict__ m_dev,
                    const void* __restrict__ image, float* __restrict__ rgb,
                    float* __restrict__ H1, float* __restrict__ H2, unsigned long long* __restrict__ masks, int experiment) {
  const int64_t M = m_dev ? (*m_dev < M_cap ? *m_dev : M_cap) : M_cap;
  constexpr int T = WIDTH / 32;
  __shared__ __attribute__((aligned(16))) X3Lds<WIDTH, KS1> L;
  x3_copy_image<X3Img<WIDTH, KS1>>(&L, image);
  __syncthreads();
  const int lane = threadIdx.x & 63, h = lane >> 5;
  float* stage = L.stage[threadIdx.x >> 6];
  const bool train = H1 != nullptr;
  const int64_t n_tiles = (M + 31) / 32;
  const int64_t gw = (int64_t)blockIdx.x * (blockDim.x >> 6) + (threadIdx.x >> 6);
  const int64_t nw = (int64_t)gridDim.x * (blockDim.x >> 6);
  const int d_in = n_view + E;
  const int64_t last = M > 0 ? M - 1 : 0;
  auto row_of = [&](int64_t tile) { const int64_t r = tile * 32 + (lane & 31); return r < M ? r : last; };
  float xin[KS1][8];
  auto load_inputs = [&](int64_t tile, int64_t rid) {
    const float* fr = feat + row_of(tile) * C + c_view0;
    const float* er = emb + rid * E - n_view;
#pragma unroll
    for (int s = 0; s < KS1; ++s)
#pragma unroll
      for (int j = 0; j < 8; ++j) {
        const int k = 16 * s + 8 * h + j;
        const int kc = k < d_in ? k : d_in - 1;
        xin[s][j] = *((kc < n_view) ? fr + kc : er + kc);
      }
  };
  int64_t rid_n = 0;
  if (gw < n_tiles) { load_inputs(gw, ray_id[row_of(gw)]); rid_n = ray_id[row_of(gw + nw)]; }
  for (int64_t tile = gw; tile < n_tiles; tile += nw) {
    const int64_t row = tile * 32 + (lane & 31);
    const bool valid = row < M;
    const int rows_valid = (int)(M - tile * 32 < 32 ? M - tile * 32 : 32);
    u32x4 x3[KS1][3];
#pragma unroll
    for (int s = 0; s < KS1; ++s) {
      float v[8];
#pragma unroll
      for (int j = 0; j < 8; ++j) v[j] = (16 * s + 8 * h + j) < d_in ? xin[s][j] : 0.0f;
      x3_split8(v, x3[s][0], x3[s][1], x3[s][2]);
    }
    load_inputs(tile + nw, rid_n);
    rid_n = ray_id[row_of(tile + 2 * nw)];
    u32x4 h3[2 * T][3];
    unsigned long long mask1 = 0ull;
#pragma unroll
    for (int t = 0; t < T; ++t) {
      f32x16 acc;
#pragma unroll
      for (int r = 0; r < 16; ++r) acc[r] = L.b1p[h][t * 16 + r];
#pragma unroll
      for (int s = 0; s < KS1; ++s)
        x3_mfma6(acc, L.w1s[t][s][0][lane], L.w1s[t][s][1][lane], L.w1s[t][s][2][lane], x3[s][0], x3[s][1], x3[s][2]);
#pragma unroll
      for (int r = 0; r < 16; ++r) acc[r] = dvgo_relu(acc[r]);
      if (train) {
        unsigned int bits = 0u;
#pragma unroll
        for (int r = 0; r < 16; ++r) bits |= dvgo_relu_bit(acc[r]) << r;
        mask1 |= (unsigned long long)bits << (16 * t);
        if (!(experiment & 512)) x3_store_tile(stage, acc, H1 + tile * 32 * WIDTH + 32 * t, WIDTH, lane, rows_valid);
      }
#pragma unroll
      for (int s2 = 0; s2 < 2; ++s2) {
        float v[8];
#pragma unroll
        for (int j = 0; j < 8; ++j) v[j] = acc[8 * s2 + j];
        x3_split8(v, h3[2 * t + s2][0], h3[2 * t + s2][1], h3[2 * t + s2][2]);
      }
      __builtin_amdgcn_sched_barrier(0);
    }
    float p[3] = {0.0f, 0.0f, 0.0f};
    unsigned long long mask2 = 0ull;
#pragma unroll 1
    for (int t2 = 0; t2 < T; ++t2) {
      f32x16 acc2;
#pragma unroll
      for (int r = 0; r < 16; ++r) acc2[r] = L.b2p[h][t2 * 16 + r];
      u32x4 a[2][3];
#pragma unroll
      for (int q = 0; q < 3; ++q) a[0][q] = L.w2s[t2][0][q][lane];
#pragma unroll
      for (int ks = 0; ks < 2 * T; ++ks) {
        if (ks + 1 < 2 * T) {
#pragma unroll
          for (int q = 0; q < 3; ++q) a[(ks + 1) & 1][q] = L.w2s[t2][ks + 1][q][lane];
        }
        x3_mfma6(acc2, a[ks & 1][0], a[ks & 1][1], a[ks & 1][2], h3[ks][0], h3[ks][1], h3[ks][2]);
        __builtin_amdgcn_sched_barrier(0);
      }
#pragma unroll
      for (int r = 0; r < 16; ++r) acc2[r] = dvgo_relu(acc2[r]);
      if (train) {
        unsigned int bits = 0u;
#pragma unroll
        for (int r = 0; r < 16; ++r) bits |= dvgo_relu_bit(acc2[r]) << r;
        mask2 |= (unsigned long long)bits << (16 * t2);
        if (!(experiment & 512)) x3_store_tile(stage, acc2, H2 + tile * 32 * WIDTH + 32 * t2, WIDTH, lane, rows_valid);
      }
#pragma unroll
      for (int c = 0; c < 3; ++c) {
#pragma unroll
        for (int r = 0; r < 16; ++r) p[c] = fmaf(L.w3p[c][h][t2 * 16 + r], acc2[r], p[c]);
      }
    }
    float z[3];
#pragma unroll
    for (int c = 0; c < 3; ++c) z[c] = p[c] + __shfl_xor(p[c], 32) + L.b3[c];
    if (valid) {
      if (h == 0) {
#pragma unroll
        for (int c = 0; c < 3; ++c) {
          const float zz = DIFFUSE ? z[c] + feat[row * C + c] : z[c];
          rgb[row * 3 + c] = 1.0f / (1.0f + expf(-zz));
        }
      }
      if (train) {
        masks[(row * 2 + 0) * 2 + h] = mask1;
        masks[(row * 2 + 1) * 2 + h] = mask2;
      }
    }
  }
}

template <int WIDTH>
struct X3BwdImg {
  static constexpr int T = WIDTH / 32;
  u32x4 w2t[T][2 * T][3][64];
  u32x4 w1t[2 * T][3][64];
  float w3p[3][2][T * 16];
};

template <int WIDTH>
struct X3BwdLds : X3BwdImg<WIDTH> {
  float stage[X3_BWD_WAVES][X3_STAGE_ROWS * X3_STAGE_STRIDE];
};

template <int WIDTH>
__device__ __forceinline__ void
x3_prep_bwd_body(X3BwdImg<WIDTH>* __restrict__ Lp, const float* __restrict__ W1, const float* __restrict__ W2,
                 const float* __restrict__ W3, int D_in, const int tid, const int nt) {
  constexpr int T = WIDTH / 32;
  X3BwdImg<WIDTH>& L = *Lp;
  for (int i = tid; i < T * 2 * T * 64 * 8; i += nt) {
    const int j = i & 7, l = (i >> 3) & 63, ks = (i >> 9) % (2 * T), tin = (i >> 9) / (2 * T);
    const int f_out = 16 * ks + 8 * (j >> 2) + 4 * (l >> 5) + (j & 3);
    unsigned short p0, p1, p2;
    x3_split1(W2[f_out * WIDTH + 32 * tin + (l & 31)], p0, p1, p2);
    reinterpret_cast<unsigned short*>(&L.w2t[tin][ks][0][l])[j] = p0;
    reinterpret_cast<unsigned short*>(&L.w2t[tin][ks][1][l])[j] = p1;
    reinterpret_cast<unsigned short*>(&L.w2t[tin][ks][2][l])[j] = p2;
  }
  for (int i = tid; i < 2 * T * 64 * 8; i += nt) {
    const int j = i & 7, l = (i >> 3) & 63, ks = i >> 9;
    const int f = 16 * ks + 8 * (j >> 2) + 4 * (l >> 5) + (j & 3), k = l & 31;
    unsigned short p0, p1, p2;
    x3_split1((k < D_in) ? W1[f * D_in + k] : 0.0f, p0, p1, p2);
    reinterpret_cast<unsigned short*>(&L.w1t[ks][0][l])[j] = p0;
    reinterpret_cast<unsigned short*>(&L.w1t[ks][1][l])[j] = p1;
    reinterpret_cast<unsigned short*>(&L.w1t[ks][2][l])[j] = p2;
  }
  for (int i = tid; i < 3 * 2 * T * 16; i += nt) {
    const int tr = i % (T * 16), h = (i / (T * 16)) & 1, c = i / (2 * T * 16);
    (&L.w3p[0][0][0])[i] = W3[c * WIDTH + x3_acc_feature(tr >> 4, tr & 15, h)];
  }
}

template <int WIDTH, int KS1>
__global__ void __launch_bounds__(256)
x3_prep_fwd_kernel(X3Img<WIDTH, KS1>* __restrict__ Lp, X3BwdImg<WIDTH>* __restrict__ Lb, const float* __restrict__ W1,
                   const float* __restrict__ b1, const float* __restrict__ W2, const float* __restrict__ b2,
                   const float* __restrict__ W3, const float* __restrict__ b3, int D_in) {
  if (blockIdx.x < 32) x3_prep_fwd_body<WIDTH, KS1>(Lp, W1, b1, W2, b2, W3, b3, D_in, blockIdx.x * blockDim.x + threadIdx.x, 32 * blockDim.x);
  else x3_prep_bwd_body<WIDTH>(Lb, W1, W2, W3, D_in, (blockIdx.x - 32) * blockDim.x + threadIdx.x, 32 * blockDim.x);
}

template <int WIDTH>
__global__ void __launch_bounds__(256)
x3_prep_bwd_kernel(X3BwdImg<WIDTH>* __restrict__ Lp, const float* __restrict__ W1, const float* __restrict__ W2,
                   const float* __restrict__ W3, int D_in) {
  x3_prep_bwd_body<WIDTH>(Lp, W1, W2, W3, D_in, blockIdx.x * blockDim.x + threadIdx.x, gridDim.x * blockDim.x);
}

template <int WIDTH, bool DIFFUSE>
__global__ void __launch_bounds__(X3_BWD_THREADS)
shade_bwd_x3_kernel(const float* __restrict__ g_rgb, const float* __restrict__ rgb,
                    const unsigned long long* __restrict__ masks, int64_t M_cap, const int64_t* __restrict__ m_dev,
                    const void* __restrict__ image, int C, int c_view0,
                    int n_view, float* __restrict__ g_feat, float* __restrict__ G1, float* __restrict__ gz_out) {
  const int64_t M = m_dev ? (*m_dev < M_cap ? *m_dev : M_cap) : M_cap;
  constexpr int T = WIDTH / 32;
  __shared__ __attribute__((aligned(16))) X3BwdLds<WIDTH> L;
  x3_copy_image<X3BwdImg<WIDTH>>(&L, image);
  __syncthreads();
  const int lane = threadIdx.x & 63, h = lane >> 5;
  float* stage = L.stage[threadIdx.x >> 6];
  const int64_t n_tiles = (M + 31) / 32;
  const int64_t gw = (int64_t)blockIdx.x * (blockDim.x >> 6) + (threadIdx.x >> 6);
  const int64_t nw = (int64_t)gridDim.x * (blockDim.x >> 6);
  const int64_t last = M > 0 ? M - 1 : 0;
  float o_n[3], g_n[3];
  unsigned long long m1_n = 0ull, m2_n = 0ull;
  auto load_rows = [&](int64_t tile) {
    const int64_t r = tile * 32 + (lane & 31);
    const int64_t rc = r < M ? r : last;
#pragma unroll
    for (int c = 0; c < 3; ++c) { o_n[c] = rgb[rc * 3 + c]; g_n[c] = g_rgb[rc * 3 + c]; }
    m1_n = masks[(rc * 2 + 0) * 2 + h];
    m2_n = masks[(rc * 2 + 1) * 2 + h];
  };
  if (gw < n_tiles) load_rows(gw);
  for (int64_t tile = gw; tile < n_tiles; tile += nw) {
    const int64_t row = tile * 32 + (lane & 31);
    const bool valid = row < M;
    const int rows_valid = (int)(M - tile * 32 < 32 ? M - tile * 32 : 32);
    float gz[3];
#pragma unroll
    for (int c = 0; c < 3; ++c) gz[c] = valid ? g_n[c] * o_n[c] * (1.0f - o_n[c]) : 0.0f;
    const unsigned long long m1 = m1_n, m2 = m2_n;
    load_rows(tile + nw);
    if (valid && h == 0) {
#pragma unroll
      for (int c = 0; c < 3; ++c) {
        gz_out[row * 3 + c] = gz[c];
        if (DIFFUSE) g_feat[row * C + c] = gz[c];
      }
    }
    u32x4 g3[2 * T][3];
#pragma unroll
    for (int t2 = 0; t2 < T; ++t2) {
#pragma unroll
      for (int s2 = 0; s2 < 2; ++s2) {
        float v[8];
#pragma unroll
        for (int j = 0; j < 8; ++j) {
          const int r = 8 * s2 + j;
          const float w = fmaf(L.w3p[2][h][t2 * 16 + r], gz[2],
                               fmaf(L.w3p[1][h][t2 * 16 + r], gz[1], L.w3p[0][h][t2 * 16 + r] * gz[0]));
          v[j] = ((m2 >> (16 * t2 + r)) & 1ull) ? w : 0.0f;
        }
        x3_split8(v, g3[2 * t2 + s2][0], g3[2 * t2 + s2][1], g3[2 * t2 + s2][2]);
      }
    }
    f32x16 gx;
#pragma unroll
    for (int r = 0; r < 16; ++r) gx[r] = 0.0f;
#pragma unroll 1
    for (int tin = 0; tin < T; ++tin) {
      f32x16 acc;
#pragma unroll
      for (int r = 0; r < 16; ++r) acc[r] = 0.0f;
#pragma unroll
      for (int ks = 0; ks < 2 * T; ++ks) {
        x3_mfma6(acc, L.w2t[tin][ks][0][lane], L.w2t[tin][ks][1][lane], L.w2t[tin][ks][2][lane], g3[ks][0], g3[ks][1], g3[ks][2]);
        if (ks & 1) __builtin_amdgcn_sched_barrier(0);
      }
#pragma unroll
      for (int q = 0; q < 4; ++q) {
        const unsigned int mb = (unsigned int)(m1 >> (16 * tin + 4 * q)) & 15u;
        acc[4 * q + 0] = (mb & 1u) ? acc[4 * q + 0] : 0.0f;
        acc[4 * q + 1] = (mb & 2u) ? acc[4 * q + 1] : 0.0f;
        acc[4 * q + 2] = (mb & 4u) ? acc[4 * q + 2] : 0.0f;
        acc[4 * q + 3] = (mb & 8u) ? acc[4 * q + 3] : 0.0f;
      }
      x3_store_tile(stage, acc, G1 + tile * 32 * WIDTH + 32 * tin, WIDTH, lane, rows_valid);
#pragma unroll
      for (int s2 = 0; s2 < 2; ++s2) {
        float v[8];
#pragma unroll
        for (int j = 0; j < 8; ++j) v[j] = acc[8 * s2 + j];
        u32x4 b0, b1, b2;
        x3_split8(v, b0, b1, b2);
        const int ks = 2 * tin + s2;
        x3_mfma6(gx, L.w1t[ks][0][lane], L.w1t[ks][1][lane], L.w1t[ks][2][lane], b0, b1, b2);
      }
    }
    if (valid) {
#pragma unroll
      for (int r = 0; r < 16; ++r) {
        const int k = (r & 3) + 8 * (r >> 2) + 4 * h;
        if (k < n_view) g_feat[row * C + c_view0 + k] = gx[r];
      }
    }
  }
}

template <int WIDTH>
struct X3WgradLds {
  static constexpr int T = WIDTH / 32;
  float g1[2][32][WIDTH], h1[2][32][WIDTH], h2[2][32][WIDTH];
  float x[2][32][40];
  float gz[2][32][4];
  unsigned int m2[2][32][2][2];
  u32x4 fb[T + 1][2][3][64];
};

typedef const __attribute__((address_space(1))) void* x3_gptr_t;
typedef __attribute__((address_space(3))) void* x3_lptr_t;

template <int WIDTH>
__global__ void __launch_bounds__(WIDTH * 4)
shade_wgrad_x3_kernel(const float* __restrict__ G1, const float* __restrict__ gz, const unsigned int* __restrict__ masks,
                      const float* __restrict__ W3, const float* __restrict__ H1, const float* __restrict__ H2,
                      const float* __restrict__ feat, int C, int c_view0, int n_view, const float* __restrict__ emb, int E,
                      const int64_t* __restrict__ ray_id, int64_t M_cap, const int64_t* __restrict__ m_dev,
                      float* __restrict__ part ) {
  const int64_t M = m_dev ? (*m_dev < M_cap ? *m_dev : M_cap) : M_cap;
  constexpr int T = WIDTH / 32;
  constexpr int NW = 2 * T;
  constexpr int NT = NW * 64;
  constexpr int TPR = NT / 32;
  constexpr int NXI = 40 / TPR > 0 ? (40 + TPR - 1) / TPR : 1;
  constexpr int LPR = WIDTH / 4;
  constexpr int RPI = 64 / LPR;
  constexpr int IPW = 32 / RPI / NW;
  __shared__ __attribute__((aligned(16))) X3WgradLds<WIDTH> L;
  const int tid = threadIdx.x, lane = tid & 63, h = lane >> 5, i = lane & 31, w = tid >> 6;
  const int ot = w >> 1, ks = w & 1;
  f32x16 aW2[T], aW1;
#pragma unroll
  for (int t = 0; t < T; ++t)
#pragma unroll
    for (int r = 0; r < 16; ++r) aW2[t][r] = 0.0f;
#pragma unroll
  for (int r = 0; r < 16; ++r) aW1[r] = 0.0f;
  float vW3[3] = {0.0f, 0.0f, 0.0f}, vW1[8];
#pragma unroll
  for (int kk = 0; kk < 8; ++kk) vW1[kk] = 0.0f;
  float sb1 = 0.0f, sb2 = 0.0f, gz_acc = 0.0f;
  const float w30 = W3[32 * ot + i], w31 = W3[WIDTH + 32 * ot + i], w32 = W3[2 * WIDTH + 32 * ot + i];
  const int m_half = (i >> 2) & 1, m_word = ot >> 1, m_bit = 16 * (ot & 1) + (i & 3) + 4 * (i >> 3);
  const int d_in = n_view + E;
  const int64_t n_tiles = (M + 31) / 32;

  float px[NXI], pgz;
  unsigned int pm2;
  bool pvalid, pgvalid;
  const int xrow = tid / TPR, xcol = tid - xrow * TPR;
  auto issue = [&](int64_t tile, int buf) {
    const int64_t r0 = tile * 32;
    {
      const int64_t row = r0 + xrow;
      const int64_t rc = row < M ? row : M - 1;
      const float* fr = feat + rc * C + c_view0;
      const float* er = emb + ray_id[rc] * E - n_view;
#pragma unroll
      for (int q = 0; q < NXI; ++q) {
        const int k = xcol + TPR * q;
        const int kc = k < d_in ? k : d_in - 1;
        px[q] = *((kc < n_view) ? fr + kc : er + kc);
      }
      pvalid = row < M;
    }
    {
      const int64_t row = r0 + ((tid & 127) >> 2);
      const int64_t rc = row < M ? row : M - 1;
      pgz = gz[rc * 3 + ((tid & 3) < 3 ? (tid & 3) : 0)];
      pgvalid = (tid & 3) < 3 && row < M;
      pm2 = masks[rc * 8 + 4 + (tid & 3)];
    }
#pragma unroll
    for (int q = 0; q < IPW; ++q) {
      const int rl = (IPW * w + q) * RPI;
      const int64_t row = r0 + rl + lane / LPR;
      const int64_t off = (row < M ? row : M - 1) * WIDTH + 4 * (lane % LPR);
      __builtin_amdgcn_global_load_lds((x3_gptr_t)(G1 + off), (x3_lptr_t)&L.g1[buf][rl][0], 16, 0, 0);
      __builtin_amdgcn_global_load_lds((x3_gptr_t)(H1 + off), (x3_lptr_t)&L.h1[buf][rl][0], 16, 0, 0);
      __builtin_amdgcn_global_load_lds((x3_gptr_t)(H2 + off), (x3_lptr_t)&L.h2[buf][rl][0], 16, 0, 0);
    }
  };

  int buf = 0;
  if ((int64_t)blockIdx.x < n_tiles) issue(blockIdx.x, 0);
  for (int64_t tile = blockIdx.x; tile < n_tiles; tile += gridDim.x, buf ^= 1) {
#pragma unroll
    for (int q = 0; q < NXI; ++q) {
      const int k = xcol + TPR * q;
      if (k < 40) L.x[buf][xrow][k] = (pvalid && k < d_in) ? px[q] : 0.0f;
    }
    if (tid < 128) {
      gz_acc += pgvalid ? pgz : 0.0f;
      L.gz[buf][tid >> 2][tid & 3] = pgvalid ? pgz : 0.0f;
      (&L.m2[buf][tid >> 2][0][0])[tid & 3] = pm2;
    }
    __builtin_amdgcn_s_waitcnt(0x0F70);
    __syncthreads();
    if (tile + gridDim.x < n_tiles) issue(tile + gridDim.x, buf ^ 1);
    const int rows_valid = (int)(M - tile * 32 < 32 ? M - tile * 32 : 32);
    {
      const int bt = w & (T - 1), bs = w / T;
      float v[8];
#pragma unroll
      for (int e = 0; e < 8; ++e) v[e] = L.h1[buf][16 * bs + 8 * h + e][32 * bt + i];
      u32x4 p0, p1, p2;
      x3_split8(v, p0, p1, p2);
      L.fb[bt][bs][0][lane] = p0; L.fb[bt][bs][1][lane] = p1; L.fb[bt][bs][2][lane] = p2;
      if (w < 2) {
#pragma unroll
        for (int e = 0; e < 8; ++e) v[e] = L.x[buf][16 * w + 8 * h + e][i];
        x3_split8(v, p0, p1, p2);
        L.fb[T][w][0][lane] = p0; L.fb[T][w][1][lane] = p1; L.fb[T][w][2][lane] = p2;
      }
    }
    u32x4 a2f[3], a1f[3];
    {
      float a2[8], a1[8];
#pragma unroll
      for (int e = 0; e < 8; ++e) {
        const int row = 16 * ks + 8 * h + e;
        const float4 gzr = *reinterpret_cast<const float4*>(&L.gz[buf][row][0]);
        const float g2v = fmaf(w32, gzr.z, fmaf(w31, gzr.y, w30 * gzr.x));
        a2[e] = ((L.m2[buf][row][m_half][m_word] >> m_bit) & 1u) ? g2v : 0.0f;
        a1[e] = row < rows_valid ? L.g1[buf][row][32 * ot + i] : 0.0f;
        sb2 += a2[e]; sb1 += a1[e];
        const float hv = L.h2[buf][row][32 * ot + i];
        vW3[0] = fmaf(gzr.x, hv, vW3[0]); vW3[1] = fmaf(gzr.y, hv, vW3[1]); vW3[2] = fmaf(gzr.z, hv, vW3[2]);
        const float4 xa = *reinterpret_cast<const float4*>(&L.x[buf][row][32]);
        const float4 xb = *reinterpret_cast<const float4*>(&L.x[buf][row][36]);
        vW1[0] = fmaf(a1[e], xa.x, vW1[0]); vW1[1] = fmaf(a1[e], xa.y, vW1[1]); vW1[2] = fmaf(a1[e], xa.z, vW1[2]);
        vW1[3] = fmaf(a1[e], xa.w, vW1[3]); vW1[4] = fmaf(a1[e], xb.x, vW1[4]); vW1[5] = fmaf(a1[e], xb.y, vW1[5]);
        vW1[6] = fmaf(a1[e], xb.z, vW1[6]); vW1[7] = fmaf(a1[e], xb.w, vW1[7]);
        if (e & 1) __builtin_amdgcn_sched_barrier(0);
      }
      x3_split8(a2, a2f[0], a2f[1], a2f[2]);
      x3_split8(a1, a1f[0], a1f[1], a1f[2]);
    }
    __syncthreads();
#pragma unroll
    for (int t = 0; t < T; ++t) {
      x3_mfma6(aW2[t], a2f[0], a2f[1], a2f[2], L.fb[t][ks][0][lane], L.fb[t][ks][1][lane], L.fb[t][ks][2][lane]);
      __builtin_amdgcn_sched_barrier(0);
    }
    x3_mfma6(aW1, a1f[0], a1f[1], a1f[2], L.fb[T][ks][0][lane], L.fb[T][ks][1][lane], L.fb[T][ks][2][lane]);
    __builtin_amdgcn_sched_barrier(0);
  }
  __syncthreads();
  float* red = &L.g1[0][0][0];
  if (ks == 1) {
#pragma unroll
    for (int t = 0; t < T; ++t)
#pragma unroll
      for (int r = 0; r < 16; ++r) red[((ot * (T + 1) + t) * 16 + r) * 64 + lane] = aW2[t][r];
#pragma unroll
    for (int r = 0; r < 16; ++r) red[((ot * (T + 1) + T) * 16 + r) * 64 + lane] = aW1[r];
  }
  static_assert((T * (T + 1) * 16 * 64 + T * 14 * 64) * 4 <= 3 * 2 * 32 * WIDTH * 4, "the exchange fits the operand buffers");
  float* red2 = red + T * (T + 1) * 16 * 64;
  if (ks == 1) {
#pragma unroll
    for (int kk = 0; kk < 8; ++kk) red2[(ot * 14 + kk) * 64 + lane] = vW1[kk];
#pragma unroll
    for (int c = 0; c < 3; ++c) red2[(ot * 14 + 8 + c) * 64 + lane] = vW3[c];
    red2[(ot * 14 + 11) * 64 + lane] = sb1;
    red2[(ot * 14 + 12) * 64 + lane] = sb2;
  }
  __syncthreads();
  float* p = part + (int64_t)blockIdx.x * (WIDTH * WIDTH + WIDTH * 64 + 32 * WIDTH + 3 * WIDTH);
  float* pW2 = p;
  float* pW1 = pW2 + WIDTH * WIDTH;
  float* pW3 = pW1 + WIDTH * 64;
  float* pb = pW3 + 32 * WIDTH;
  if (ks == 0) {
#pragma unroll
    for (int r = 0; r < 16; ++r) {
      const int oi = (r & 3) + 8 * (r >> 2) + 4 * h;
#pragma unroll
      for (int t = 0; t < T; ++t)
        pW2[(32 * ot + oi) * WIDTH + 32 * t + i] = aW2[t][r] + red[((ot * (T + 1) + t) * 16 + r) * 64 + lane];
      pW1[(32 * ot + oi) * 64 + i] = aW1[r] + red[((ot * (T + 1) + T) * 16 + r) * 64 + lane];
    }
#pragma unroll
    for (int kk = 0; kk < 8; ++kk) {
      float v = vW1[kk] + red2[(ot * 14 + kk) * 64 + lane];
      v += __shfl_xor(v, 32);
      if (h == 0) pW1[(32 * ot + i) * 64 + 32 + kk] = v;
    }
    if (h == 0) {
#pragma unroll
      for (int kk = 8; kk < 32; ++kk) pW1[(32 * ot + i) * 64 + 32 + kk] = 0.0f;
    }
#pragma unroll
    for (int c = 0; c < 3; ++c) {
      float v = vW3[c] + red2[(ot * 14 + 8 + c) * 64 + lane];
      v += __shfl_xor(v, 32);
      if (h == 0) pW3[c * WIDTH + 32 * ot + i] = v;
    }
    float s1 = sb1 + red2[(ot * 14 + 11) * 64 + lane], s2 = sb2 + red2[(ot * 14 + 12) * 64 + lane];
    s1 += __shfl_xor(s1, 32); s2 += __shfl_xor(s2, 32);
    if (h == 0) { pb[32 * ot + i] = s1; pb[WIDTH + 32 * ot + i] = s2; }
  }
  float gz_sum = gz_acc;
  gz_sum += __shfl_xor(gz_sum, 4); gz_sum += __shfl_xor(gz_sum, 8);
  gz_sum += __shfl_xor(gz_sum, 16); gz_sum += __shfl_xor(gz_sum, 32);
  if (w < 2 && lane < 3) pb[2 * WIDTH + 8 * w + lane] = gz_sum;
  for (int q = tid; q < WIDTH; q += NT)
    if (q >= 16 || (q & 7) >= 3) pb[2 * WIDTH + q] = 0.0f;
}

template <int WIDTH>
struct X3WgradLdsB {
  static constexpr int T = WIDTH / 32;
  float g1[32][WIDTH], h1[32][WIDTH];
  float x[32][40];
  float gz[32][4];
  unsigned int m2[32][2][2];
  u32x4 fb[T + 1][2][3][64];
};

template <int WIDTH>
__global__ void __launch_bounds__(WIDTH * 2, 2)
shade_wgrad_x3b_kernel(const float* __restrict__ G1, const float* __restrict__ gz, const unsigned int* __restrict__ masks,
                       const float* __restrict__ W3, const float* __restrict__ H1, const float* __restrict__ H2,
                       const float* __restrict__ feat, int C, int c_view0, int n_view, const float* __restrict__ emb, int E,
                       const int64_t* __restrict__ ray_id, int64_t M_cap, const int64_t* __restrict__ m_dev,
                       float* __restrict__ part ) {
  const int64_t M = m_dev ? (*m_dev < M_cap ? *m_dev : M_cap) : M_cap;
  constexpr int T = WIDTH / 32;
  constexpr int NW = T;
  constexpr int NT = NW * 64;
  constexpr int TPR = NT / 32;
  constexpr int NXI = (40 + TPR - 1) / TPR;
  constexpr int LPR = WIDTH / 4;
  constexpr int RPI = 64 / LPR;
  constexpr int IPW = 32 / RPI / NW;
  __shared__ __attribute__((aligned(16))) X3WgradLdsB<WIDTH> L;
  static_assert(sizeof(X3WgradLdsB<WIDTH>) <= 80 * 1024, "two workgroups per CU");
  const int tid = threadIdx.x, lane = tid & 63, h = lane >> 5, i = lane & 31, w = tid >> 6;
  const int ot = w;
  f32x16 aW2[T], aW1;
#pragma unroll
  for (int t = 0; t < T; ++t)
#pragma unroll
    for (int r = 0; r < 16; ++r) aW2[t][r] = 0.0f;
#pragma unroll
  for (int r = 0; r < 16; ++r) aW1[r] = 0.0f;
  float vW3[3] = {0.0f, 0.0f, 0.0f}, vW1[8];
#pragma unroll
  for (int kk = 0; kk < 8; ++kk) vW1[kk] = 0.0f;
  float sb1 = 0.0f, sb2 = 0.0f, gz_acc = 0.0f;
  const float w30 = W3[32 * ot + i], w31 = W3[WIDTH + 32 * ot + i], w32 = W3[2 * WIDTH + 32 * ot + i];
  const int m_half = (i >> 2) & 1, m_word = ot >> 1, m_bit = 16 * (ot & 1) + (i & 3) + 4 * (i >> 3);
  const int d_in = n_view + E;
  const int64_t n_tiles = (M + 31) / 32;
  const int xrow = tid / TPR, xcol = tid - xrow * TPR;

  for (int64_t tile = blockIdx.x; tile < n_tiles; tile += gridDim.x) {
    const int64_t r0 = tile * 32;
#pragma unroll
    for (int q = 0; q < IPW; ++q) {
      const int rl = (IPW * w + q) * RPI;
      const int64_t row = r0 + rl + lane / LPR;
      const int64_t off = (row < M ? row : M - 1) * WIDTH + 4 * (lane % LPR);
      __builtin_amdgcn_global_load_lds((x3_gptr_t)(G1 + off), (x3_lptr_t)&L.g1[rl][0], 16, 0, 0);
      __builtin_amdgcn_global_load_lds((x3_gptr_t)(H1 + off), (x3_lptr_t)&L.h1[rl][0], 16, 0, 0);
    }
    {
      const int64_t row = r0 + xrow;
      const int64_t rc = row < M ? row : M - 1;
      const float* fr = feat + rc * C + c_view0;
      const float* er = emb + ray_id[rc] * E - n_view;
#pragma unroll
      for (int q = 0; q < NXI; ++q) {
        const int k = xcol + TPR * q;
        const int kc = k < d_in ? k : d_in - 1;
        const float v = *((kc < n_view) ? fr + kc : er + kc);
        if (k < 40) L.x[xrow][k] = (row < M && k < d_in) ? v : 0.0f;
      }
    }
    if (tid < 128) {
      const int64_t row = r0 + (tid >> 2);
      const int64_t rc = row < M ? row : M - 1;
      const bool ok = (tid & 3) < 3 && row < M;
      const float g = gz[rc * 3 + ((tid & 3) < 3 ? (tid & 3) : 0)];
      gz_acc += ok ? g : 0.0f;
      L.gz[tid >> 2][tid & 3] = ok ? g : 0.0f;
      (&L.m2[tid >> 2][0][0])[tid & 3] = masks[rc * 8 + 4 + (tid & 3)];
    }
    __builtin_amdgcn_s_waitcnt(0x0F70);
    __syncthreads();
    const int rows_valid = (int)(M - r0 < 32 ? M - r0 : 32);
    {
      u32x4 p0, p1, p2;
      float v[8];
#pragma unroll
      for (int bs = 0; bs < 2; ++bs) {
#pragma unroll
        for (int e = 0; e < 8; ++e) v[e] = L.h1[16 * bs + 8 * h + e][32 * w + i];
        x3_split8(v, p0, p1, p2);
        L.fb[w][bs][0][lane] = p0; L.fb[w][bs][1][lane] = p1; L.fb[w][bs][2][lane] = p2;
      }
      if (w < 2) {
#pragma unroll
        for (int e = 0; e < 8; ++e) v[e] = L.x[16 * w + 8 * h + e][i];
        x3_split8(v, p0, p1, p2);
        L.fb[T][w][0][lane] = p0; L.fb[T][w][1][lane] = p1; L.fb[T][w][2][lane] = p2;
      }
    }
    __syncthreads();
#pragma unroll 1
    for (int ks = 0; ks < 2; ++ks) {
      u32x4 a2f[3], a1f[3];
      {
        float hv[8];
#pragma unroll
        for (int e = 0; e < 8; ++e) {
          const int64_t row = r0 + 16 * ks + 8 * h + e;
          hv[e] = H2[(row < M ? row : M - 1) * WIDTH + 32 * ot + i];
        }
        float a2[8], a1[8];
#pragma unroll
        for (int e = 0; e < 8; ++e) {
          const int row = 16 * ks + 8 * h + e;
          const float4 gzr = *reinterpret_cast<const float4*>(&L.gz[row][0]);
          const float g2v = fmaf(w32, gzr.z, fmaf(w31, gzr.y, w30 * gzr.x));
          a2[e] = ((L.m2[row][m_half][m_word] >> m_bit) & 1u) ? g2v : 0.0f;
          a1[e] = row < rows_valid ? L.g1[row][32 * ot + i] : 0.0f;
          sb2 += a2[e]; sb1 += a1[e];
          vW3[0] = fmaf(gzr.x, hv[e], vW3[0]); vW3[1] = fmaf(gzr.y, hv[e], vW3[1]); vW3[2] = fmaf(gzr.z, hv[e], vW3[2]);
          const float4 xa = *reinterpret_cast<const float4*>(&L.x[row][32]);
          const float4 xb = *reinterpret_cast<const float4*>(&L.x[row][36]);
          vW1[0] = fmaf(a1[e], xa.x, vW1[0]); vW1[1] = fmaf(a1[e], xa.y, vW1[1]); vW1[2] = fmaf(a1[e], xa.z, vW1[2]);
          vW1[3] = fmaf(a1[e], xa.w, vW1[3]); vW1[4] = fmaf(a1[e], xb.x, vW1[4]); vW1[5] = fmaf(a1[e], xb.y, vW1[5]);
          vW1[6] = fmaf(a1[e], xb.z, vW1[6]); vW1[7] = fmaf(a1[e], xb.w, vW1[7]);
          if (e & 1) __builtin_amdgcn_sched_barrier(0);
        }
        x3_split8(a2, a2f[0], a2f[1], a2f[2]);
        x3_split8(a1, a1f[0], a1f[1], a1f[2]);
      }
#pragma unroll
      for (int t = 0; t < T; ++t) {
        x3_mfma6(aW2[t], a2f[0], a2f[1], a2f[2], L.fb[t][ks][0][lane], L.fb[t][ks][1][lane], L.fb[t][ks][2][lane]);
        __builtin_amdgcn_sched_barrier(0);
      }
      x3_mfma6(aW1, a1f[0], a1f[1], a1f[2], L.fb[T][ks][0][lane], L.fb[T][ks][1][lane], L.fb[T][ks][2][lane]);
      __builtin_amdgcn_sched_barrier(0);
    }
    __syncthreads();
  }
  float* p = part + (int64_t)blockIdx.x * (WIDTH * WIDTH + WIDTH * 64 + 32 * WIDTH + 3 * WIDTH);
  float* pW2 = p;
  float* pW1 = pW2 + WIDTH * WIDTH;
  float* pW3 = pW1 + WIDTH * 64;
  float* pb = pW3 + 32 * WIDTH;
#pragma unroll
  for (int r = 0; r < 16; ++r) {
    const int oi = (r & 3) + 8 * (r >> 2) + 4 * h;
#pragma unroll
    for (int t = 0; t < T; ++t) pW2[(32 * ot + oi) * WIDTH + 32 * t + i] = aW2[t][r];
    pW1[(32 * ot + oi) * 64 + i] = aW1[r];
  }
#pragma unroll
  for (int kk = 0; kk < 8; ++kk) {
    float v = vW1[kk];
    v += __shfl_xor(v, 32);
    if (h == 0) pW1[(32 * ot + i) * 64 + 32 + kk] = v;
  }
  if (h == 0) {
#pragma unroll
    for (int kk = 8; kk < 32; ++kk) pW1[(32 * ot + i) * 64 + 32 + kk] = 0.0f;
  }
#pragma unroll
  for (int c = 0; c < 3; ++c) {
    float v = vW3[c];
    v += __shfl_xor(v, 32);
    if (h == 0) pW3[c * WIDTH + 32 * ot + i] = v;
  }
  float s1 = sb1, s2 = sb2;
  s1 += __shfl_xor(s1, 32); s2 += __shfl_xor(s2, 32);
  if (h == 0) { pb[32 * ot + i] = s1; pb[WIDTH + 32 * ot + i] = s2; }
  float gz_sum = gz_acc;
  gz_sum += __shfl_xor(gz_sum, 4); gz_sum += __shfl_xor(gz_sum, 8);
  gz_sum += __shfl_xor(gz_sum, 16); gz_sum += __shfl_xor(gz_sum, 32);
  if (w < 2 && lane < 3) pb[2 * WIDTH + 8 * w + lane] = gz_sum;
  for (int q = tid; q < WIDTH; q += NT)
    if (q >= 16 || (q & 7) >= 3) pb[2 * WIDTH + q] = 0.0f;
}

typedef __attribute__((ext_vector_type(3))) unsigned int u32x3;
typedef __attribute__((ext_vector_type(2))) unsigned int u32x2;

#define X3C_PART(W) ((W) * (W) + (W) * 64 + 32 * (W) + 3 * (W))

template <int WIDTH, int EXP = 0>
__global__ void __launch_bounds__(WIDTH * 2, 2)
shade_wgrad_c2_kernel(const float* __restrict__ gz, const unsigned int* __restrict__ masks, const float* __restrict__ W3,
                      const float* __restrict__ H1, const float* __restrict__ H2, int64_t M_cap,
                      const int64_t* __restrict__ m_dev, float* __restrict__ part) {
#if defined(__HIP_DEVICE_COMPILE__)
  const int64_t M = m_dev ? (*m_dev < M_cap ? *m_dev : M_cap) : M_cap;
  constexpr int T = WIDTH / 32;
  const int lane = threadIdx.x & 63, h = lane >> 5, i = lane & 31;
  const int ot = __builtin_amdgcn_readfirstlane(threadIdx.x >> 6);
  const unsigned int Mu = (unsigned int)M;
  const auto bH1 = __builtin_amdgcn_make_buffer_rsrc((void*)H1, 0, Mu * (WIDTH * 4u), 0x00020000);
  const auto bH2 = __builtin_amdgcn_make_buffer_rsrc((void*)H2, 0, Mu * (WIDTH * 4u), 0x00020000);
  const auto bGz = __builtin_amdgcn_make_buffer_rsrc((void*)gz, 0, Mu * 12u, 0x00020000);
  const auto bM = __builtin_amdgcn_make_buffer_rsrc((void*)masks, 0, Mu * 32u, 0x00020000);
  f32x16 aW2[T];
#pragma unroll
  for (int t = 0; t < T; ++t)
#pragma unroll
    for (int r = 0; r < 16; ++r) aW2[t][r] = 0.0f;
  float vW3[3] = {0.0f, 0.0f, 0.0f}, g3[3] = {0.0f, 0.0f, 0.0f}, sb2 = 0.0f;
  const float w30 = W3[32 * ot + i], w31 = W3[WIDTH + 32 * ot + i], w32 = W3[2 * WIDTH + 32 * ot + i];
  const unsigned int m_bit = 16 * (ot & 1) + (i & 3) + 4 * (i >> 3);
  int vo_h = (8 * h * WIDTH + i) * 4;
  int vo_hw = (8 * h * WIDTH + T * i) * 4;
  int vo_gz = 8 * h * 12;
  int vo_m = (8 * h * 8 + 4 + 2 * ((i >> 2) & 1) + (ot >> 1)) * 4;
  const int n_ks = (int)((M + 15) >> 4);
  float rh1[T][8], rh2[8];
  u32x3 rgz[8];
  unsigned int rm[8];
  auto ld_small = [&](int k) {
#pragma unroll
    for (int e = 0; e < 8; ++e) {
      rgz[e] = __builtin_amdgcn_raw_buffer_load_b96(bGz, vo_gz + e * 12, k * (16 * 12), 0);
      rm[e] = __builtin_amdgcn_raw_buffer_load_b32(bM, vo_m + e * 32, k * (16 * 32), 0);
      rh2[e] = __builtin_bit_cast(float, __builtin_amdgcn_raw_buffer_load_b32(bH2, vo_h + e * (WIDTH * 4), k * (16 * WIDTH * 4) + ot * 128, 0));
    }
  };
  auto ld_h1 = [&](int e, int k) {
    if constexpr (T == 4) {
      const u32x4 v = __builtin_amdgcn_raw_buffer_load_b128(bH1, vo_hw + e * (WIDTH * 4), k * (16 * WIDTH * 4), 0);
#pragma unroll
      for (int t = 0; t < T; ++t) rh1[t][e] = __uint_as_float(v[t]);
    } else {
      const u32x2 v = __builtin_amdgcn_raw_buffer_load_b64(bH1, vo_hw + e * (WIDTH * 4), k * (16 * WIDTH * 4), 0);
#pragma unroll
      for (int t = 0; t < T; ++t) rh1[t][e] = __uint_as_float(v[t]);
    }
  };
  int ks = blockIdx.x;
  if (ks < n_ks) {
    __builtin_amdgcn_sched_barrier(0);
    ld_small(ks);
    __builtin_amdgcn_sched_barrier(0);
#pragma unroll
    for (int e = 0; e < 8; ++e) ld_h1(e, ks);
    __builtin_amdgcn_sched_barrier(0);
  }
  for (; ks < n_ks; ks += gridDim.x) {
    const int kn = ks + (int)gridDim.x < n_ks ? ks + (int)gridDim.x : n_ks - 1;
    asm volatile("" : "+v"(vo_h), "+v"(vo_hw), "+v"(vo_gz), "+v"(vo_m));
    float a2[8];
#pragma unroll
    for (int e = 0; e < 8; ++e) {
      const float g0 = __uint_as_float(rgz[e][0]), g1 = __uint_as_float(rgz[e][1]), g2 = __uint_as_float(rgz[e][2]);
      const float g2v = fmaf(w32, g2, fmaf(w31, g1, w30 * g0));
      a2[e] = __uint_as_float(__float_as_uint(g2v) & (unsigned int)__builtin_amdgcn_sbfe((int)rm[e], m_bit, 1u));
      sb2 += a2[e];
      const float hv = rh2[e];
      vW3[0] = fmaf(g0, hv, vW3[0]); vW3[1] = fmaf(g1, hv, vW3[1]); vW3[2] = fmaf(g2, hv, vW3[2]);
    }
    if (ot == 0) {
      asm volatile("" : "+v"(g3[0]), "+v"(g3[1]), "+v"(g3[2]));
#pragma unroll
      for (int e = 0; e < 8; ++e) {
        g3[0] += __uint_as_float(rgz[e][0]); g3[1] += __uint_as_float(rgz[e][1]); g3[2] += __uint_as_float(rgz[e][2]);
      }
    }
    asm volatile("" : "+v"(a2[0]), "+v"(a2[1]), "+v"(a2[2]), "+v"(a2[3]), "+v"(a2[4]), "+v"(a2[5]), "+v"(a2[6]), "+v"(a2[7]),
                      "+v"(vW3[0]), "+v"(vW3[1]), "+v"(vW3[2]), "+v"(sb2), "+v"(g3[0]), "+v"(g3[1]), "+v"(g3[2]));
    if (!(EXP & 2)) ld_small(kn);
    __builtin_amdgcn_sched_barrier(0);
    u32x4 a2f[3];
    x3_split8(a2, a2f[0], a2f[1], a2f[2]);
    u32x4 bf[2][3];
    {
      float v[8];
#pragma unroll
      for (int e = 0; e < 8; ++e) v[e] = rh1[0][e];
      x3_split8_free(v, bf[0][0], bf[0][1], bf[0][2]);
    }
#pragma unroll
    for (int t = 0; t < T; ++t) {
      if (t + 1 < T) {
        float v[8];
#pragma unroll
        for (int e = 0; e < 8; ++e) v[e] = rh1[t + 1][e];
        if (!(EXP & 4)) x3_split8_free(v, bf[(t + 1) & 1][0], bf[(t + 1) & 1][1], bf[(t + 1) & 1][2]);
        else {
#pragma unroll
          for (int q = 0; q < 3; ++q)
#pragma unroll
            for (int c = 0; c < 4; ++c) bf[(t + 1) & 1][q][c] = __float_as_uint(v[(c + q) & 7]) ^ __float_as_uint(v[c + 4]);
        }
      }
      if (!(EXP & 1)) x3_mfma6(aW2[t], a2f[0], a2f[1], a2f[2], bf[t & 1][0], bf[t & 1][1], bf[t & 1][2]);
      else { aW2[t][0] += __uint_as_float(bf[t & 1][0][0] ^ bf[t & 1][1][1] ^ bf[t & 1][2][2] ^ a2f[0][0] ^ a2f[1][0] ^ a2f[2][0]); }
      if (t + 1 < T) {
#pragma unroll
        for (int g = 0; g < 6; ++g) {
          __builtin_amdgcn_sched_group_barrier(0x008, 1, 0);
          __builtin_amdgcn_sched_group_barrier(0x002, 8, 0);
        }
      }
      __builtin_amdgcn_sched_barrier(0);
      if (t + 2 == T) {
        asm volatile("" : "+v"(bf[(t + 1) & 1][0]), "+v"(bf[(t + 1) & 1][1]), "+v"(bf[(t + 1) & 1][2]));
        if (!(EXP & 2)) {
#pragma unroll
          for (int e = 0; e < 8; ++e) ld_h1(e, kn);
        }
        __builtin_amdgcn_sched_barrier(0);
      }
    }
  }
  float* p = part + (int64_t)blockIdx.x * X3C_PART(WIDTH);
  float* pW2 = p;
  float* pW3 = pW2 + WIDTH * WIDTH + WIDTH * 64;
  float* pb = pW3 + 32 * WIDTH;
#pragma unroll
  for (int r = 0; r < 16; ++r) {
    const int oi = (r & 3) + 8 * (r >> 2) + 4 * h;
#pragma unroll
    for (int t = 0; t < T; ++t) pW2[(32 * ot + oi) * WIDTH + T * i + t] = aW2[t][r];
  }
#pragma unroll
  for (int c = 0; c < 3; ++c) {
    float v = vW3[c];
    v += __shfl_xor(v, 32);
    if (h == 0) pW3[c * WIDTH + 32 * ot + i] = v;
  }
  float s2 = sb2;
  s2 += __shfl_xor(s2, 32);
  if (h == 0) pb[WIDTH + 32 * ot + i] = s2;
  if (ot == 0) {
#pragma unroll
    for (int c = 0; c < 3; ++c) {
      const float v = g3[c] + __shfl_xor(g3[c], 32);
      if (lane == 0) pb[2 * WIDTH + c] = v;
    }
  }
  for (int q = threadIdx.x; q < WIDTH; q += WIDTH * 2)
    if (q >= 3) pb[2 * WIDTH + q] = 0.0f;
#endif
}

template <int WIDTH>
__global__ void __launch_bounds__(256, 2)
shade_wgrad_c1_kernel(const float* __restrict__ G1, const float* __restrict__ feat, int C, int c_view0, int n_view,
                      const float* __restrict__ emb, int E, const int64_t* __restrict__ ray_id, int64_t M_cap,
                      const int64_t* __restrict__ m_dev, float* __restrict__ part) {
#if defined(__HIP_DEVICE_COMPILE__)
  const int64_t M = m_dev ? (*m_dev < M_cap ? *m_dev : M_cap) : M_cap;
  constexpr int T = WIDTH / 32, TA = T / 2;
  __shared__ float red[2][TA * 2 * 16 * 64 + 64 * TA];
  const int lane = threadIdx.x & 63, h = lane >> 5, i = lane & 31;
  const int w = __builtin_amdgcn_readfirstlane(threadIdx.x >> 6);
  const int half = w & 1, grp = w >> 1;
  const unsigned int Mu = (unsigned int)M;
  const auto bG1 = __builtin_amdgcn_make_buffer_rsrc((void*)G1, 0, Mu * (WIDTH * 4u), 0x00020000);
  const auto bF = __builtin_amdgcn_make_buffer_rsrc((void*)feat, 0, Mu * (unsigned int)(C * 4), 0x00020000);
  const auto bE = __builtin_amdgcn_make_buffer_rsrc((void*)emb, 0, 0x80000000u, 0x00020000);
  const auto bR = __builtin_amdgcn_make_buffer_rsrc((void*)ray_id, 0, Mu * 8u, 0x00020000);
  f32x16 aW1[TA][2];
  float sb1[TA];
#pragma unroll
  for (int t = 0; t < TA; ++t) {
    sb1[t] = 0.0f;
#pragma unroll
    for (int q = 0; q < 2; ++q)
#pragma unroll
      for (int r = 0; r < 16; ++r) aW1[t][q][r] = 0.0f;
  }
  const int d_in = n_view + E;
  const bool from_feat = i < n_view;
  const int kf = i < n_view ? i : (n_view > 0 ? n_view - 1 : 0);
  const int ke0 = (i < n_view ? n_view : (i < d_in ? i : d_in - 1)) - n_view;
  const int ke1 = (32 + i < d_in ? 32 + i : d_in - 1) - n_view;
  int vo_g = (8 * h * WIDTH + T * i + TA * half) * 4;
  int vo_f = (8 * h * C + c_view0 + kf) * 4;
  int vo_r = 8 * h * 8;
  const int n_ks = (int)((M + 15) >> 4);
  const int stride = 2 * (int)gridDim.x;
  float rg[TA][8], rf[8], re0[8], re1[8];
  int rid[8];
  auto ld_rid = [&](int k) {
#pragma unroll
    for (int e = 0; e < 8; ++e) rid[e] = __builtin_amdgcn_raw_buffer_load_b32(bR, vo_r + e * 8, k * (16 * 8), 0);
  };
  auto ld_g = [&](int k) {
#pragma unroll
    for (int e = 0; e < 8; ++e) {
      if constexpr (TA == 2) {
        const u32x2 v = __builtin_amdgcn_raw_buffer_load_b64(bG1, vo_g + e * (WIDTH * 4), k * (16 * WIDTH * 4), 0);
        rg[0][e] = __uint_as_float(v[0]); rg[1][e] = __uint_as_float(v[1]);
      } else {
        rg[0][e] = __builtin_bit_cast(float, __builtin_amdgcn_raw_buffer_load_b32(bG1, vo_g + e * (WIDTH * 4), k * (16 * WIDTH * 4), 0));
      }
    }
  };
  auto ld_x = [&](int k) {
#pragma unroll
    for (int e = 0; e < 8; ++e) {
      rf[e] = __builtin_bit_cast(float, __builtin_amdgcn_raw_buffer_load_b32(bF, vo_f + e * (C * 4), k * (16 * C * 4), 0));
      const int vo_e = rid[e] * (E * 4);
      re0[e] = __builtin_bit_cast(float, __builtin_amdgcn_raw_buffer_load_b32(bE, vo_e + ke0 * 4, 0, 0));
      re1[e] = __builtin_bit_cast(float, __builtin_amdgcn_raw_buffer_load_b32(bE, vo_e + ke1 * 4, 0, 0));
    }
  };
  auto clampk = [&](int k) { return k < n_ks ? k : (n_ks > 0 ? n_ks - 1 : 0); };
  int ks = 2 * (int)blockIdx.x + grp;
  if (ks < n_ks) {
    __builtin_amdgcn_sched_barrier(0);
    ld_rid(ks);
    __builtin_amdgcn_sched_barrier(0);
    ld_g(ks);
    __builtin_amdgcn_sched_barrier(0);
    ld_x(ks);
    __builtin_amdgcn_sched_barrier(0);
    ld_rid(clampk(ks + stride));
    __builtin_amdgcn_sched_barrier(0);
  }
  for (; ks < n_ks; ks += stride) {
    const int kn = clampk(ks + stride), kn2 = clampk(ks + 2 * stride);
    asm volatile("" : "+v"(vo_g), "+v"(vo_f), "+v"(vo_r));
    u32x4 af[TA][3];
#pragma unroll
    for (int t = 0; t < TA; ++t) {
      float a1[8];
#pragma unroll
      for (int e = 0; e < 8; ++e) { a1[e] = rg[t][e]; sb1[t] += a1[e]; }
      x3_split8_free(a1, af[t][0], af[t][1], af[t][2]);
    }
    if constexpr (TA == 2)
      asm volatile("" : "+v"(af[0][0]), "+v"(af[0][1]), "+v"(af[0][2]), "+v"(af[1][0]), "+v"(af[1][1]), "+v"(af[1][2]), "+v"(sb1[0]), "+v"(sb1[1]));
    else
      asm volatile("" : "+v"(af[0][0]), "+v"(af[0][1]), "+v"(af[0][2]), "+v"(sb1[0]));
    ld_g(kn);
    __builtin_amdgcn_sched_barrier(0);
    u32x4 b0, b1, b2, c0, c1, c2;
    {
      float x0[8], x1[8];
#pragma unroll
      for (int e = 0; e < 8; ++e) { x0[e] = from_feat ? rf[e] : re0[e]; x1[e] = re1[e]; }
      x3_split8(x0, b0, b1, b2);
      x3_split8(x1, c0, c1, c2);
    }
    asm volatile("" : "+v"(b0), "+v"(b1), "+v"(b2), "+v"(c0), "+v"(c1), "+v"(c2));
    ld_x(kn);
    __builtin_amdgcn_sched_barrier(0);
    ld_rid(kn2);
    __builtin_amdgcn_sched_barrier(0);
#pragma unroll
    for (int t = 0; t < TA; ++t) {
      x3_mfma6(aW1[t][0], af[t][0], af[t][1], af[t][2], b0, b1, b2);
      x3_mfma6(aW1[t][1], af[t][0], af[t][1], af[t][2], c0, c1, c2);
    }
  }
  if (grp == 1) {
#pragma unroll
    for (int t = 0; t < TA; ++t) {
#pragma unroll
      for (int q = 0; q < 2; ++q)
#pragma unroll
        for (int r = 0; r < 16; ++r) red[half][((t * 2 + q) * 16 + r) * 64 + lane] = aW1[t][q][r];
      red[half][TA * 2 * 16 * 64 + 64 * t + lane] = sb1[t];
    }
  }
  __syncthreads();
  if (grp == 0) {
    float* p = part + (int64_t)blockIdx.x * X3C_PART(WIDTH);
    float* pW1 = p + WIDTH * WIDTH;
    float* pb = pW1 + WIDTH * 64 + 32 * WIDTH;
#pragma unroll
    for (int t = 0; t < TA; ++t) {
      const int tile = TA * half + t;
#pragma unroll
      for (int r = 0; r < 16; ++r) {
        const int oi = (r & 3) + 8 * (r >> 2) + 4 * h;
#pragma unroll
        for (int q = 0; q < 2; ++q)
          pW1[(T * oi + tile) * 64 + 32 * q + i] = aW1[t][q][r] + red[half][((t * 2 + q) * 16 + r) * 64 + lane];
      }
      float s1 = sb1[t] + red[half][TA * 2 * 16 * 64 + 64 * t + lane];
      s1 += __shfl_xor(s1, 32);
      if (h == 0) pb[T * i + tile] = s1;
    }
  }
#endif
}

extern "C" {

int64_t dvgo_shade_scratch_bytes(int width) {
  if (width == 128) return (int64_t)sizeof(X3Img<128, 3>) > (int64_t)sizeof(X3BwdImg<128>) ? sizeof(X3Img<128, 3>) : sizeof(X3BwdImg<128>);
  if (width == 64) return (int64_t)sizeof(X3Img<64, 3>) > (int64_t)sizeof(X3BwdImg<64>) ? sizeof(X3Img<64, 3>) : sizeof(X3BwdImg<64>);
  return 0;
}

int dvgo_shade_fwd_x3(const float* feat, int C, const float* emb, int E, const int64_t* ray_id, int64_t M, const int64_t* m_dev,
                      const float* W1, const float* b1, const float* W2, const float* b2, const float* W3,
                      const float* b3, int width, int d_in, int diffuse, float* rgb, float* H1, float* H2,
                      uint64_t* masks, void* scratch, void* scratch_bwd, int experiment, void* stream) {
  if (M < 0 || C <= 0 || E < 0) return DVGO_EINVAL;
  if (M == 0) return 0;
  if (!feat || !emb || !ray_id || !W1 || !b1 || !W2 || !b2 || !W3 || !b3 || !rgb || !scratch) return DVGO_EINVAL;
  if ((H1 == nullptr) != (H2 == nullptr) || (H1 == nullptr) != (masks == nullptr)) return DVGO_EINVAL;
  const int c_view0 = diffuse ? 3 : 0;
  const int n_view = C - c_view0;
  if (n_view < 0 || d_in != n_view + E) return DVGO_EINVAL;
  if ((width != 128 && width != 64) || d_in > 48) return DVGO_ERANGE;
  hipStream_t s = (hipStream_t)stream;
  const int64_t n_tiles = (M + 31) / 32;
  const int64_t cap = 256;
  const int blocks = (int)((n_tiles + X3_WAVES - 1) / X3_WAVES < cap ? (n_tiles + X3_WAVES - 1) / X3_WAVES : cap);
#define DVGO_SHADE_X3(W, KS, DIFF)                                                                                       \
  do {                                                                                                                   \
    x3_prep_fwd_kernel<W, KS><<<scratch_bwd ? 64 : 32, 256, 0, s>>>((X3Img<W, KS>*)scratch, (X3BwdImg<W>*)scratch_bwd, W1, b1, W2, b2, W3, b3, d_in); \
    shade_fwd_x3_kernel<W, KS, DIFF><<<blocks, X3_THREADS, 0, s>>>(feat, C, c_view0, n_view, emb, E, ray_id, M, m_dev, scratch, rgb, \
                                                                    H1, H2, (unsigned long long*)masks, experiment);     \
  } while (0)
  if (width == 128) {
    if (diffuse) DVGO_SHADE_X3(128, 3, true); else DVGO_SHADE_X3(128, 3, false);
  } else {
    if (d_in <= 16) { if (diffuse) DVGO_SHADE_X3(64, 1, true); else DVGO_SHADE_X3(64, 1, false); }
    else            { if (diffuse) DVGO_SHADE_X3(64, 3, true); else DVGO_SHADE_X3(64, 3, false); }
  }
#undef DVGO_SHADE_X3
  DVGO_LAUNCH_CHECK();
  return 0;
}

int dvgo_shade_bwd_x3(const float* g_rgb, const float* rgb, const uint64_t* masks, int64_t M, const int64_t* m_dev,
                      const float* W1, const float* W2, const float* W3, int width, int d_in, int C, int diffuse,
                      float* g_feat, float* G1, float* gz, void* scratch, int prebuilt, void* stream) {
  if (M < 0 || C <= 0) return DVGO_EINVAL;
  if (M == 0) return 0;
  if (!g_rgb || !rgb || !masks || !W1 || !W2 || !W3 || !g_feat || !G1 || !gz || !scratch) return DVGO_EINVAL;
  const int c_view0 = diffuse ? 3 : 0;
  const int n_view = C - c_view0;
  if ((width != 128 && width != 64) || n_view < 0 || n_view > 32 || d_in < n_view) return DVGO_ERANGE;
  hipStream_t s = (hipStream_t)stream;
  const int64_t n_tiles = (M + 31) / 32;
  const int64_t cap = 256;
  const int blocks = (int)((n_tiles + X3_BWD_WAVES - 1) / X3_BWD_WAVES < cap ? (n_tiles + X3_BWD_WAVES - 1) / X3_BWD_WAVES : cap);
#define DVGO_SHADE_BWD_X3(W, DIFF)                                                                                        \
  do {                                                                                                                    \
    if (!prebuilt) x3_prep_bwd_kernel<W><<<32, 256, 0, s>>>((X3BwdImg<W>*)scratch, W1, W2, W3, d_in);                   \
    shade_bwd_x3_kernel<W, DIFF><<<blocks, X3_BWD_THREADS, 0, s>>>(g_rgb, rgb, (const unsigned long long*)masks, M, m_dev, scratch, C, \
                                                                c_view0, n_view, g_feat, G1, gz);                         \
  } while (0)
  if (width == 128) { if (diffuse) DVGO_SHADE_BWD_X3(128, true); else DVGO_SHADE_BWD_X3(128, false); }
  else              { if (diffuse) DVGO_SHADE_BWD_X3(64, true); else DVGO_SHADE_BWD_X3(64, false); }
#undef DVGO_SHADE_BWD_X3
  DVGO_LAUNCH_CHECK();
  return 0;
}

int dvgo_shade_wgrad_x3(const float* G1, const float* gz, const uint64_t* masks, const float* W3, const float* H1,
                        const float* H2, const float* feat, int C, const float* emb, int E, const int64_t* ray_id, int64_t M,
                        const int64_t* m_dev, int width, int diffuse, int n_parts, float* part, int form_b, void* stream) {
  if (M < 0 || n_parts <= 0 || C <= 0 || E < 0) return DVGO_EINVAL;
  if (!G1 || !gz || !masks || !W3 || !H1 || !H2 || !feat || !emb || !ray_id || !part) return DVGO_EINVAL;
  const int c_view0 = diffuse ? 3 : 0;
  const int n_view = C - c_view0;
  if ((width != 128 && width != 64) || n_view < 0 || n_view + E > 40) return DVGO_ERANGE;
  if (form_b == 2) {
    if (M * width * 4 >= ((int64_t)1 << 32) || M * C * 4 >= ((int64_t)1 << 32) || M * 32 >= ((int64_t)1 << 32)) return DVGO_ERANGE;
    if (width == 128) {
      shade_wgrad_c2_kernel<128><<<n_parts, 256, 0, (hipStream_t)stream>>>(gz, (const unsigned int*)masks, W3, H1, H2, M, m_dev, part);
      shade_wgrad_c1_kernel<128><<<n_parts, 256, 0, (hipStream_t)stream>>>(G1, feat, C, c_view0, n_view, emb, E, ray_id, M, m_dev, part);
    } else {
      shade_wgrad_c2_kernel<64><<<n_parts, 128, 0, (hipStream_t)stream>>>(gz, (const unsigned int*)masks, W3, H1, H2, M, m_dev, part);
      shade_wgrad_c1_kernel<64><<<n_parts, 256, 0, (hipStream_t)stream>>>(G1, feat, C, c_view0, n_view, emb, E, ray_id, M, m_dev, part);
    }
  } else if (form_b && width == 128)
    shade_wgrad_x3b_kernel<128><<<n_parts, 256, 0, (hipStream_t)stream>>>(G1, gz, (const unsigned int*)masks, W3, H1, H2, feat, C,
                                                                          c_view0, n_view, emb, E, ray_id, M, m_dev, part);
  else if (form_b)
    shade_wgrad_x3b_kernel<64><<<n_parts, 128, 0, (hipStream_t)stream>>>(G1, gz, (const unsigned int*)masks, W3, H1, H2, feat, C,
                                                                         c_view0, n_view, emb, E, ray_id, M, m_dev, part);
  else if (width == 128)
    shade_wgrad_x3_kernel<128><<<n_parts, 512, 0, (hipStream_t)stream>>>(G1, gz, (const unsigned int*)masks, W3, H1, H2, feat, C,
                                                                         c_view0, n_view, emb, E, ray_id, M, m_dev, part);
  else
    shade_wgrad_x3_kernel<64><<<n_parts, 256, 0, (hipStream_t)stream>>>(G1, gz, (const unsigned int*)masks, W3, H1, H2, feat, C,
                                                                        c_view0, n_view, emb, E, ray_id, M, m_dev, part);
  DVGO_LAUNCH_CHECK();
  return 0;
}

}
```

directvoxgo_amd/shade.py:

```python

import torch
import torch.nn as nn

from . import _lib as L
from ._lib import _i64, _int, ptr, stream_of

N_PARTS = 512


class defer_wgrad:
    _active = None
    _streams = {}

    def __init__(self, side_stream=True):
        self.side_stream = side_stream

    def __enter__(self):
        self.pending = []
        defer_wgrad._active = self
        return self

    def __exit__(self, *exc):
        defer_wgrad._active = None
        return False

    def submit(self, params, fn, device):
        if not self.side_stream:
            self.pending.append((params, fn, None, None))
            return
        side = defer_wgrad._streams.get(device)
        if side is None:
            side = defer_wgrad._streams[device] = torch.cuda.Stream(device=device)
        main = torch.cuda.current_stream(device)
        side.wait_stream(main)
        with torch.cuda.stream(side):
            grads = fn()
            done = torch.cuda.Event()
            done.record(side)
        self.pending.append((params, fn, grads, done))

    @torch.no_grad()
    def flush(self):
        for params, fn, grads, done in self.pending:
            if grads is None:
                grads = fn()
            else:
                torch.cuda.current_stream(grads[0].device).wait_event(done)
            for p, g in zip(params, grads):
                if p.requires_grad:
                    p.grad = g if p.grad is None else p.grad + g
        self.pending = []


@torch.no_grad()
def viewdir_embed(viewdirs, viewfreq):
    N, F = viewdirs.shape[0], viewfreq.shape[0]
    emb = torch.empty((N, 3 + 6 * F), dtype=torch.float32, device=viewdirs.device)
    with L.device_of(viewdirs):
        L.call('dvgo_viewdir_embed', ptr(viewdirs.contiguous()), ptr(viewfreq), _int(F), _i64(N), ptr(emb),
               stream_of(viewdirs))
    return emb


def head_layers(rgbnet):
    layers = head_layers_any_din(rgbnet)
    if layers is None or layers[0].in_features > 40:
        return None
    return layers


def _scratch(width, device):
    lib = L.lib()
    n = int(lib.dvgo_shade_scratch_bytes(int(width)))
    return torch.empty(n, dtype=torch.uint8, device=device) if n > 0 else None


def _unpack_record(tot, width, d_in):
    o = 0
    gW2 = tot[o:o + width * width].view(width, width); o += width * width
    gW1 = tot[o:o + width * d_in].view(width, d_in); o += width * d_in
    gW3 = tot[o:o + 3 * width].view(3, width); o += 3 * width
    gb1, gb2, gb3 = tot[o:o + width], tot[o + width:o + 2 * width], tot[o + 2 * width:o + 2 * width + 3]
    return gW1, gb1, gW2, gb2, gW3, gb3


def _weight_grads(params, wgrad, device, k, n, g_first=None):
    grads = [g_first] + [None] * (n - 1)
    if defer_wgrad._active is not None:
        defer_wgrad._active.submit(params, wgrad, device)
    else:
        grads[k:k + 6] = wgrad()
    return tuple(grads)


class _Shade(torch.autograd.Function):
    @staticmethod
    def forward(ctx, feat, emb, ray_id, W1, b1, W2, b2, W3, b3, diffuse, train, m_dev):
        M, C = feat.shape
        E = emb.shape[1]
        width, d_in = W1.shape
        feat, emb = feat.contiguous(), emb.contiguous()
        train = bool(train) and any(ctx.needs_input_grad)
        rgb = torch.empty((M, 3), dtype=torch.float32, device=feat.device)
        H1 = torch.empty((M, width), dtype=torch.float32, device=feat.device) if train else None
        H2 = torch.empty((M, width), dtype=torch.float32, device=feat.device) if train else None
        masks = torch.empty((M, 4), dtype=torch.int64, device=feat.device) if train else None
        scratch = _scratch(width, feat.device)
        scratch_bwd = _scratch(width, feat.device) if (train and (L.lib().dvgo_shade_variant(-1) & 2)) else None
        with L.device_of(feat):
            L.call('dvgo_shade_fwd', ptr(feat), _int(C), ptr(emb), _int(E), ptr(ray_id), _i64(M), ptr(m_dev), ptr(W1.contiguous()),
                   ptr(b1.contiguous()), ptr(W2.contiguous()), ptr(b2.contiguous()), ptr(W3.contiguous()),
                   ptr(b3.contiguous()), _int(width), _int(d_in), _int(1 if diffuse else 0), ptr(rgb), ptr(H1), ptr(H2),
                   ptr(masks), ptr(scratch), ptr(scratch_bwd), stream_of(feat))
        ctx.scratch_bwd = scratch_bwd if (train and (L.lib().dvgo_shade_variant(-1) & 1)) else None
        if train:
            ctx.save_for_backward(feat, emb, ray_id, W1, W2, W3, rgb, H1, H2, masks)
            ctx.diffuse = diffuse
            ctx.m_dev = m_dev
            ctx.params = (W1, b1, W2, b2, W3, b3)
            ctx.w_versions = (W1._version, W2._version, W3._version)
        return rgb

    @staticmethod
    @torch.autograd.function.once_differentiable
    def backward(ctx, g_rgb):
        feat, emb, ray_id, W1, W2, W3, rgb, H1, H2, masks = ctx.saved_tensors
        diffuse, m_dev = ctx.diffuse, ctx.m_dev
        M, C = feat.shape
        width, d_in = W1.shape
        g_feat = torch.empty_like(feat)
        G1 = torch.empty_like(H1)
        gz = torch.empty_like(rgb)
        prebuilt = ctx.scratch_bwd is not None and W1._version == ctx.w_versions[0] and W2._version == ctx.w_versions[1] \
            and W3._version == ctx.w_versions[2]
        scratch = ctx.scratch_bwd if prebuilt else _scratch(width, feat.device)
        ctx.scratch_bwd = None
        with L.device_of(feat):
            L.call('dvgo_shade_bwd', ptr(g_rgb.contiguous()), ptr(rgb), ptr(masks), _i64(M), ptr(m_dev), ptr(W1.contiguous()),
                   ptr(W2.contiguous()), ptr(W3.contiguous()), _int(width), _int(d_in), _int(C), _int(1 if diffuse else 0),
                   ptr(g_feat), ptr(G1), ptr(gz), ptr(scratch), _int(1 if prebuilt else 0), stream_of(feat))

        def wgrad():
            n_parts = max(1, min(N_PARTS, (M + 255) // 256))
            psize = width * width + width * 64 + 32 * width + 3 * width
            part = torch.empty((n_parts, psize), dtype=torch.float32, device=feat.device)
            tsize = width * width + width * d_in + 5 * width + 3
            tot = torch.empty(tsize, dtype=torch.float32, device=feat.device)
            with L.device_of(feat):
                L.call('dvgo_shade_wgrad', ptr(G1), ptr(gz), ptr(masks), ptr(W3.contiguous()), ptr(H1), ptr(H2), ptr(feat), _int(C), ptr(emb),
                       _int(emb.shape[1]), ptr(ray_id), _i64(M), ptr(m_dev), _int(width), _int(1 if diffuse else 0), _int(n_parts),
                       ptr(part), ptr(tot), stream_of(feat))
            return _unpack_record(tot, width, d_in)

        return _weight_grads(ctx.params, wgrad, feat.device, 3, 12, g_feat if ctx.needs_input_grad[0] else None)


def shade(rgbnet, feat, emb, ray_id, diffuse, m_dev=None):
    layers = head_layers(rgbnet)
    if layers is None or not feat.is_cuda:
        return None
    l1, l2, l3 = layers
    c0 = 3 if diffuse else 0
    if l1.in_features != feat.shape[1] - c0 + emb.shape[1]:
        return None
    return _Shade.apply(feat, emb, ray_id, l1.weight, l1.bias, l2.weight, l2.bias, l3.weight, l3.bias, diffuse,
                        torch.is_grad_enabled(), m_dev)


def posenc_supported(rgbnet, n_freq, emb_dim):
    layers = head_layers_any_din(rgbnet)
    return (layers is not None and layers[0].out_features == 128 and 1 <= n_freq
            and layers[0].in_features == 3 + 6 * n_freq + emb_dim <= 96)


def head_layers_any_din(rgbnet):
    if not isinstance(rgbnet, nn.Sequential) or len(rgbnet) != 4:
        return None
    a, r, mid, c = rgbnet
    if not (isinstance(a, nn.Linear) and isinstance(r, nn.ReLU) and isinstance(c, nn.Linear)):
        return None
    if not (isinstance(mid, nn.Sequential) and len(mid) == 2 and isinstance(mid[0], nn.Linear) and isinstance(mid[1], nn.ReLU)):
        return None
    width = a.out_features
    if width not in (128, 64) or mid[0].in_features != width or mid[0].out_features != width or c.in_features != width \
            or c.out_features != 3:
        return None
    return a, mid[0], c


class _ShadePosenc(torch.autograd.Function):

    @staticmethod
    def forward(ctx, pts, emb, ray_id, freq, W1, b1, W2, b2, W3, b3, train):
        M = pts.shape[0]
        P, E = freq.shape[0], emb.shape[1]
        width, d_in = W1.shape
        pts, emb, freq = pts.contiguous(), emb.contiguous(), freq.contiguous()
        train = bool(train) and any(ctx.needs_input_grad)
        dev = pts.device
        rgb = torch.empty((M, 3), dtype=torch.float32, device=dev)
        H1 = torch.empty((M, width), dtype=torch.float32, device=dev) if train else None
        H2 = torch.empty((M, width), dtype=torch.float32, device=dev) if train else None
        masks = torch.empty((M, 4), dtype=torch.int64, device=dev) if train else None
        with L.device_of(pts):
            L.call('dvgo_shade_pe_fwd', ptr(pts), ptr(freq), _int(P), ptr(emb), _int(E), ptr(ray_id), _i64(M), ptr(W1.contiguous()),
                   ptr(b1.contiguous()), ptr(W2.contiguous()), ptr(b2.contiguous()), ptr(W3.contiguous()), ptr(b3.contiguous()),
                   _int(width), _int(d_in), ptr(rgb), ptr(H1), ptr(H2), ptr(masks), stream_of(pts))
        if train:
            ctx.save_for_backward(pts, emb, ray_id, freq, W2, W3, rgb, H1, H2, masks)
            ctx.params = (W1, b1, W2, b2, W3, b3)
            ctx.d_in = d_in
        return rgb

    @staticmethod
    @torch.autograd.function.once_differentiable
    def backward(ctx, g_rgb):
        pts, emb, ray_id, freq, W2, W3, rgb, H1, H2, masks = ctx.saved_tensors
        M, width, d_in = pts.shape[0], H1.shape[1], ctx.d_in
        G1 = torch.empty_like(H1)
        gz = torch.empty_like(rgb)
        with L.device_of(pts):
            L.call('dvgo_shade_pe_bwd', ptr(g_rgb.contiguous()), ptr(rgb), ptr(masks), _i64(M), ptr(W2.contiguous()),
                   ptr(W3.contiguous()), _int(width), ptr(G1), ptr(gz), stream_of(pts))

        def wgrad():
            rec = int(L.lib().dvgo_shade_pe_record_size(width, d_in))
            n_parts = max(1, min(N_PARTS, (M + 31) // 32))
            part = torch.empty((n_parts, rec), dtype=torch.float32, device=pts.device)
            tot = torch.empty(rec, dtype=torch.float32, device=pts.device)
            with L.device_of(pts):
                L.call('dvgo_shade_pe_wgrad', ptr(G1), ptr(gz), ptr(masks), ptr(W3.contiguous()), ptr(H1), ptr(H2), ptr(pts),
                       ptr(freq), _int(freq.shape[0]), ptr(emb), _int(emb.shape[1]), ptr(ray_id), _i64(M), _int(width),
                       _int(d_in), _int(n_parts), ptr(part), ptr(tot), stream_of(pts))
            return _unpack_record(tot, width, d_in)

        return _weight_grads(ctx.params, wgrad, pts.device, 4, 11)


def shade_posenc(rgbnet, pts, emb, ray_id, posfreq):
    if not pts.is_cuda or not posenc_supported(rgbnet, posfreq.shape[0], emb.shape[1]):
        return None
    l1, l2, l3 = head_layers_any_din(rgbnet)
    return _ShadePosenc.apply(pts, emb, ray_id, posfreq, l1.weight, l1.bias, l2.weight, l2.bias, l3.weight, l3.bias,
                              torch.is_grad_enabled())


@torch.no_grad()
def march_positions(start, dirs, ray_id, step_id, stepdist):
    M = ray_id.shape[0]
    pts = torch.empty((M, 3), dtype=torch.float32, device=start.device)
    with L.device_of(start):
        L.call('dvgo_march_positions', ptr(start), ptr(dirs), ptr(ray_id), ptr(step_id), _i64(M), L._flt(float(stepdist)), ptr(pts),
               stream_of(start))
    return pts
```

Baseline: 3.160 million.

## Store shading MLP activations in a tiled record layout shared across passes

Adds a 'record' mode in which the forward, backward and weight-gradient shading kernels keep H1, H2 and G1 in one contiguous buffer, laid out in 16-row tiles with interleaved 8-float groups. The forward and backward kernels write activations straight from registers with float4 stores, skipping the LDS staging area and its per-wave buffer. The wgrad kernels read through remapped offsets. This is meant to cut LDS use and staging overhead and make the stores coalesce better. It adds padding to multiples of 32 rows and a new layout that every consumer has to decode correctly.

```diff
diff --git a/directvoxgo_amd/csrc/shade.hip b/directvoxgo_amd/csrc/shade.hip
--- a/directvoxgo_amd/csrc/shade.hip
+++ b/directvoxgo_amd/csrc/shade.hip
@@ -5,19 +5,19 @@
 
 
 static int g_shade_experiment = 0;
-static int g_shade_variant = 67;
+static int g_shade_variant = 195;
 extern "C" int dvgo_shade_wgrad_x3(const float* G1, const float* gz, const uint64_t* masks, const float* W3, const float* H1,
                                    const float* H2, const float* feat, int C, const float* emb, int E, const int64_t* ray_id,
                                    int64_t M, const int64_t* m_dev, int width, int diffuse, int n_parts, float* part, int form_b,
                                    void* stream);
 extern "C" int dvgo_shade_bwd_x3(const float* g_rgb, const float* rgb, const uint64_t* masks, int64_t M, const int64_t* m_dev,
                                  const float* W1, const float* W2, const float* W3, int width, int d_in, int C, int diffuse,
-                                 float* g_feat, float* G1, float* gz, void* scratch, int prebuilt, void* stream);
+                                 float* g_feat, float* G1, float* gz, void* scratch, int prebuilt, int record, void* stream);
 
 extern "C" int dvgo_shade_fwd_x3(const float* feat, int C, const float* emb, int E, const int64_t* ray_id, int64_t M, const int64_t* m_dev,
                                  const float* W1, const float* b1, const float* W2, const float* b2, const float* W3,
                                  const float* b3, int width, int d_in, int diffuse, float* rgb, float* H1, float* H2,
-                                 uint64_t* masks, void* scratch, void* scratch_bwd, int experiment, void* stream);
+                                 uint64_t* masks, void* scratch, void* scratch_bwd, int experiment, int record, void* stream);
 
 #define SHADE_THREADS 768
 #define SHADE_WAVES (SHADE_THREADS / 64)
@@ -329,7 +329,7 @@
 typedef const __attribute__((address_space(1))) void* dvgo_gptr_t;
 typedef __attribute__((address_space(3))) void* dvgo_lptr_t;
 
-template <int WIDTH>
+template <int WIDTH, bool REC = false>
 __global__ void __launch_bounds__(2 * WIDTH) __attribute__((amdgpu_num_vgpr(104)))
 shade_wgrad_kernel(const float* __restrict__ G1, const float* __restrict__ gz, const unsigned int* __restrict__ masks,
                    const float* __restrict__ W3, const float* __restrict__ H1, const float* __restrict__ H2, const float* __restrict__ feat, int C,
@@ -400,7 +400,10 @@
     _Pragma("unroll") for (int i = 0; i < 4; ++i) {             \
       const int rl = (4 * w + i) * RPI;                  \
       const int64_t row = r0_ + rl + lane / LPR;                                                                \
-      const int64_t off = (row < M ? row : M - 1) * WIDTH + 4 * (lane % LPR);                                   \
+       \
+      const int u_ = lane % LPR;                                                                                \
+      const int64_t off = REC ? (row >> 4) * (16 * WIDTH) + ((((u_ >> 1) * 16 + (int)(row & 15)) * 2 + (u_ & 1)) * 4) \
+                              : (row < M ? row : M - 1) * WIDTH + 4 * u_;                                       \
       __builtin_amdgcn_global_load_lds((dvgo_gptr_t)(G1 + off), (dvgo_lptr_t)&L.g1[BUF][rl][0], 16, 0, 0);     \
       __builtin_amdgcn_global_load_lds((dvgo_gptr_t)(H1 + off), (dvgo_lptr_t)&L.h1[BUF][rl][0], 16, 0, 0);     \
       __builtin_amdgcn_global_load_lds((dvgo_gptr_t)(H2 + off), (dvgo_lptr_t)&L.h2[BUF][rl][0], 16, 0, 0);     \
@@ -771,7 +774,7 @@
   u32x4 fb[WIDTH / 32 + 2][3][64];
 };
 
-template <int WIDTH>
+template <int WIDTH, bool REC>
 __global__ void __launch_bounds__(2 * WIDTH, 2)
 shade_wgrad_ring_x3_kernel(const float* __restrict__ G1, const float* __restrict__ gz, const unsigned int* __restrict__ masks,
                            const float* __restrict__ W3, const float* __restrict__ H1, const float* __restrict__ H2,
@@ -812,7 +815,7 @@
   const int d_in = n_view + E;
   const int n_tiles = (int)((M + TR - 1) / TR);
   auto tile_of = [&](int k) { return (int)blockIdx.x + k * (int)gridDim.x; };
-  const unsigned rows_b = (unsigned)(M * WIDTH * 4);
+  const unsigned rows_b = (unsigned)((REC ? (M + 31) / 32 * 32 : M) * WIDTH * 4);
   const auto bG1 = __builtin_amdgcn_make_buffer_rsrc((void*)G1, 0, rows_b, 0x00020000);
   const auto bH1 = __builtin_amdgcn_make_buffer_rsrc((void*)H1, 0, rows_b, 0x00020000);
   const auto bH2 = __builtin_amdgcn_make_buffer_rsrc((void*)H2, 0, rows_b, 0x00020000);
@@ -824,7 +827,10 @@
   unsigned vo_bulk[IPW], vo_f[FPW], vo_ecol[EPW];
   int e_row[EPW];
 #pragma unroll
-  for (int i = 0; i < IPW; ++i) vo_bulk[i] = (unsigned)(((IPW * w + i) * RPI + lane / LPR) * WIDTH * 4 + 16 * (lane % LPR));
+  for (int i = 0; i < IPW; ++i) {
+    const int row = (IPW * w + i) * RPI + lane / LPR, u = lane % LPR;
+    vo_bulk[i] = REC ? (unsigned)((((u >> 1) * 16 + row) * 2 + (u & 1)) * 16) : (unsigned)(row * WIDTH * 4 + 16 * u);
+  }
 #pragma unroll
   for (int i = 0; i < FPW; ++i) {
     const int e = 64 * ((dw < 0 ? 0 : dw) + DW * i) + lane, row = e >> 4, col = e & 15;
@@ -1062,6 +1068,13 @@
   if (p1 > p0) atomicAdd(out + o, (a0 + a1) + (a2 + a3));
 }
 
+static bool shade_record_ok(int width) { return (g_shade_variant & 127) == 67 && (width == 128 || width == 64); }
+static bool shade_ring_ok(int width, int n_view, int E, int64_t M, int C) {
+  return n_view <= 16 && E <= 32 && (n_view + E <= 32 || (n_view % 4 == 0 && n_view >= 8)) &&
+         M * width * 4 < ((int64_t)1 << 31) && M * C * 4 < ((int64_t)1 << 31);
+}
+static int64_t shade_record_region(int64_t M, int width) { return (M + 31) / 32 * 32 * width; }
+
 extern "C" {
 
 int dvgo_shade_fwd(const float* feat, int C, const float* emb, int E, const int64_t* ray_id, int64_t M, const int64_t* m_dev,
@@ -1071,14 +1084,20 @@
   if (M < 0 || C <= 0 || E < 0) return DVGO_EINVAL;
   if (M == 0) return 0;
   if (!feat || !emb || !ray_id || !W1 || !b1 || !W2 || !b2 || !W3 || !b3 || !rgb) return DVGO_EINVAL;
-  if ((H1 == nullptr) != (H2 == nullptr) || (H1 == nullptr) != (masks == nullptr)) return DVGO_EINVAL;
+  const bool record = H1 != nullptr && H2 == nullptr && masks != nullptr;
+  if (!record && ((H1 == nullptr) != (H2 == nullptr) || (H1 == nullptr) != (masks == nullptr))) return DVGO_EINVAL;
   const int c_view0 = diffuse ? 3 : 0;
   const int n_view = C - c_view0;
   if (n_view < 0 || d_in != n_view + E) return DVGO_EINVAL;
   if ((width != 128 && width != 64) || d_in > 40) return DVGO_ERANGE;
+  if (record) {
+    if (!scratch || !shade_record_ok(width)) return DVGO_ERANGE;
+    return dvgo_shade_fwd_x3(feat, C, emb, E, ray_id, M, m_dev, W1, b1, W2, b2, W3, b3, width, d_in, diffuse, rgb, H1,
+                             H1 + shade_record_region(M, width), masks, scratch, scratch_bwd, g_shade_experiment, 1, stream);
+  }
   if ((g_shade_variant & 1) && scratch != nullptr)
     return dvgo_shade_fwd_x3(feat, C, emb, E, ray_id, M, m_dev, W1, b1, W2, b2, W3, b3, width, d_in, diffuse, rgb, H1, H2, masks,
-                             scratch, (g_shade_variant & 2) ? scratch_bwd : nullptr, g_shade_experiment, stream);
+                             scratch, (g_shade_variant & 2) ? scratch_bwd : nullptr, g_shade_experiment, 0, stream);
   hipStream_t s = (hipStream_t)stream;
   const int64_t n_tiles = (M + 31) / 32;
   const int64_t cap = width == 128 ? 256 : 512;
@@ -1111,8 +1130,13 @@
   const int c_view0 = diffuse ? 3 : 0;
   const int n_view = C - c_view0;
   if ((width != 128 && width != 64) || n_view < 0 || n_view > 32 || d_in < n_view) return DVGO_ERANGE;
+  if (prebuilt & 2) {
+    if (!scratch || !shade_record_ok(width)) return DVGO_ERANGE;
+    return dvgo_shade_bwd_x3(g_rgb, rgb, masks, M, m_dev, W1, W2, W3, width, d_in, C, diffuse, g_feat,
+                             G1 + 2 * shade_record_region(M, width), gz, scratch, prebuilt & 1, 1, stream);
+  }
   if ((g_shade_variant & 2) && scratch != nullptr)
-    return dvgo_shade_bwd_x3(g_rgb, rgb, masks, M, m_dev, W1, W2, W3, width, d_in, C, diffuse, g_feat, G1, gz, scratch, prebuilt, stream);
+    return dvgo_shade_bwd_x3(g_rgb, rgb, masks, M, m_dev, W1, W2, W3, width, d_in, C, diffuse, g_feat, G1, gz, scratch, prebuilt, 0, stream);
   hipStream_t s = (hipStream_t)stream;
   const int64_t n_tiles = (M + 31) / 32;
   const int64_t cap = width == 128 ? 256 : 512;
@@ -1131,27 +1155,48 @@
                      const float* H2, const float* feat, int C, const float* emb, int E, const int64_t* ray_id, int64_t M,
                      const int64_t* m_dev, int width, int diffuse, int n_parts, float* part, float* total, void* stream) {
   if (M < 0 || n_parts <= 0 || C <= 0 || E < 0) return DVGO_EINVAL;
-  if (!G1 || !gz || !masks || !W3 || !H1 || !H2 || !feat || !emb || !ray_id || !part || !total) return DVGO_EINVAL;
+  const bool record = H2 == nullptr;
+  if (!G1 || !gz || !masks || !W3 || !H1 || (!record && !H2) || !feat || !emb || !ray_id || !part || !total) return DVGO_EINVAL;
+  if (record && H1 != G1) return DVGO_EINVAL;
   const int c_view0 = diffuse ? 3 : 0;
   const int n_view = C - c_view0;
   if ((width != 128 && width != 64) || n_view < 0 || n_view + E > 40) return DVGO_ERANGE;
   bool ring = false;
-  if (g_shade_variant & (4 | 32)) {
+  if (record) {
+    if (!shade_record_ok(width)) return DVGO_ERANGE;
+    const int tsz = width * width + width * (n_view + E) + 5 * width + 3;
+    const int64_t reg = shade_record_region(M, width);
+    const float *rH1 = G1, *rH2 = G1 + reg, *rG1 = G1 + 2 * reg;
+    if (shade_ring_ok(width, n_view, E, M, C)) {
+      if (n_parts > 512) n_parts = 512;
+      ring = true;
+      if (width == 128)
+        shade_wgrad_ring_x3_kernel<128, true><<<n_parts, 256, 0, (hipStream_t)stream>>>(
+            rG1, gz, (const unsigned int*)masks, W3, rH1, rH2, feat, C, c_view0, n_view, emb, E, ray_id, M, m_dev, part, total, tsz);
+      else
+        shade_wgrad_ring_x3_kernel<64, true><<<n_parts, 128, 0, (hipStream_t)stream>>>(
+            rG1, gz, (const unsigned int*)masks, W3, rH1, rH2, feat, C, c_view0, n_view, emb, E, ray_id, M, m_dev, part, total, tsz);
+    } else if (width == 128)
+      shade_wgrad_kernel<128, true><<<n_parts, 256, 0, (hipStream_t)stream>>>(
+          rG1, gz, (const unsigned int*)masks, W3, rH1, rH2, feat, C, c_view0, n_view, emb, E, ray_id, M, m_dev, part);
+    else
+      shade_wgrad_kernel<64, true><<<n_parts, 128, 0, (hipStream_t)stream>>>(
+          rG1, gz, (const unsigned int*)masks, W3, rH1, rH2, feat, C, c_view0, n_view, emb, E, ray_id, M, m_dev, part);
+  } else if (g_shade_variant & (4 | 32)) {
     const int form_b = (g_shade_variant & 32) ? 2 : (g_shade_variant & 16) ? 1 : 0;
     if (!form_b && n_parts > 256) n_parts = 256;
     const int rc = dvgo_shade_wgrad_x3(G1, gz, masks, W3, H1, H2, feat, C, emb, E, ray_id, M, m_dev, width, diffuse, n_parts, part,
                                        form_b, stream);
     if (rc != 0) return rc;
-  } else if (!(g_shade_variant & 8) && n_view <= 16 && E <= 32 && (n_view + E <= 32 || (n_view % 4 == 0 && n_view >= 8)) &&
-             M * width * 4 < ((int64_t)1 << 31) && M * C * 4 < ((int64_t)1 << 31)) {
+  } else if (!(g_shade_variant & 8) && shade_ring_ok(width, n_view, E, M, C)) {
     if (n_parts > 512) n_parts = 512;
     ring = true;
     const int tsz = width * width + width * (n_view + E) + 5 * width + 3;
     if ((g_shade_variant & 64) && width == 128)
-      shade_wgrad_ring_x3_kernel<128><<<n_parts, 256, 0, (hipStream_t)stream>>>(
+      shade_wgrad_ring_x3_kernel<128, false><<<n_parts, 256, 0, (hipStream_t)stream>>>(
           G1, gz, (const unsigned int*)masks, W3, H1, H2, feat, C, c_view0, n_view, emb, E, ray_id, M, m_dev, part, total, tsz);
     else if (g_shade_variant & 64)
-      shade_wgrad_ring_x3_kernel<64><<<n_parts, 128, 0, (hipStream_t)stream>>>(
+      shade_wgrad_ring_x3_kernel<64, false><<<n_parts, 128, 0, (hipStream_t)stream>>>(
           G1, gz, (const unsigned int*)masks, W3, H1, H2, feat, C, c_view0, n_view, emb, E, ray_id, M, m_dev, part, total, tsz);
     else if (width == 128)
       shade_wgrad_ring_kernel<128><<<n_parts, 256, 0, (hipStream_t)stream>>>(
diff --git a/directvoxgo_amd/csrc/shade_x3.hip b/directvoxgo_amd/csrc/shade_x3.hip
--- a/directvoxgo_amd/csrc/shade_x3.hip
+++ b/directvoxgo_amd/csrc/shade_x3.hip
@@ -33,10 +33,28 @@
   float b3[4];
 };
 
-template <int WIDTH, int KS1>
+template <int WIDTH, int KS1, bool REC>
 struct X3Lds : X3Img<WIDTH, KS1> {
   float stage[X3_WAVES][X3_STAGE_ROWS * X3_STAGE_STRIDE];
 };
+template <int WIDTH, int KS1>
+struct X3Lds<WIDTH, KS1, true> : X3Img<WIDTH, KS1> {};
+
+__device__ __forceinline__ void x3_store_tile_rec(const f32x16& acc, float* __restrict__ dst , int width,
+                                                  int t, int lane, bool full, bool valid) {
+  const int smp = lane & 31, h = lane >> 5;
+  float* d = dst + (smp >> 4) * 16 * width + (4 * t * 16 + (smp & 15)) * 8 + 4 * h;
+  if (full) {
+#pragma unroll
+    for (int q = 0; q < 4; ++q)
+      *reinterpret_cast<float4*>(d + q * 128) = make_float4(acc[4 * q], acc[4 * q + 1], acc[4 * q + 2], acc[4 * q + 3]);
+  } else {
+#pragma unroll
+    for (int q = 0; q < 4; ++q)
+      *reinterpret_cast<float4*>(d + q * 128) =
+          valid ? make_float4(acc[4 * q], acc[4 * q + 1], acc[4 * q + 2], acc[4 * q + 3]) : make_float4(0.0f, 0.0f, 0.0f, 0.0f);
+  }
+}
 
 template <typename Img>
 __device__ __forceinline__ void x3_copy_image(Img* __restrict__ dst , const void* __restrict__ src) {
@@ -108,7 +126,7 @@
   if (tid < 4) L.b3[tid] = tid < 3 ? b3[tid] : 0.0f;
 }
 
-template <int WIDTH, int KS1, bool DIFFUSE>
+template <int WIDTH, int KS1, bool DIFFUSE, bool REC>
 __global__ void __launch_bounds__(X3_THREADS)
 shade_fwd_x3_kernel(const float* __restrict__ feat, int C, int c_view0, int n_view, const float* __restrict__ emb, int E,
                     const int64_t* __restrict__ ray_id, int64_t M_cap, const int64_t* __restrict__ m_dev,
@@ -116,11 +134,12 @@
                     float* __restrict__ H1, float* __restrict__ H2, unsigned long long* __restrict__ masks, int experiment) {
   const int64_t M = m_dev ? (*m_dev < M_cap ? *m_dev : M_cap) : M_cap;
   constexpr int T = WIDTH / 32;
-  __shared__ __attribute__((aligned(16))) X3Lds<WIDTH, KS1> L;
+  __shared__ __attribute__((aligned(16))) X3Lds<WIDTH, KS1, REC> L;
   x3_copy_image<X3Img<WIDTH, KS1>>(&L, image);
   __syncthreads();
   const int lane = threadIdx.x & 63, h = lane >> 5;
-  float* stage = L.stage[threadIdx.x >> 6];
+  float* stage = nullptr;
+  if constexpr (!REC) stage = L.stage[threadIdx.x >> 6];
   const bool train = H1 != nullptr;
   const int64_t n_tiles = (M + 31) / 32;
   const int64_t gw = (int64_t)blockIdx.x * (blockDim.x >> 6) + (threadIdx.x >> 6);
@@ -147,6 +166,7 @@
     const int64_t row = tile * 32 + (lane & 31);
     const bool valid = row < M;
     const int rows_valid = (int)(M - tile * 32 < 32 ? M - tile * 32 : 32);
+    const bool full = __builtin_amdgcn_readfirstlane(rows_valid) == 32;
     u32x4 x3[KS1][3];
 #pragma unroll
     for (int s = 0; s < KS1; ++s) {
@@ -174,7 +194,8 @@
 #pragma unroll
         for (int r = 0; r < 16; ++r) bits |= dvgo_relu_bit(acc[r]) << r;
         mask1 |= (unsigned long long)bits << (16 * t);
-        if (!(experiment & 512)) x3_store_tile(stage, acc, H1 + tile * 32 * WIDTH + 32 * t, WIDTH, lane, rows_valid);
+        if constexpr (REC) x3_store_tile_rec(acc, H1 + tile * 32 * WIDTH, WIDTH, t, lane, full, valid);
+        else if (!(experiment & 512)) x3_store_tile(stage, acc, H1 + tile * 32 * WIDTH + 32 * t, WIDTH, lane, rows_valid);
       }
 #pragma unroll
       for (int s2 = 0; s2 < 2; ++s2) {
@@ -211,7 +232,8 @@
 #pragma unroll
         for (int r = 0; r < 16; ++r) bits |= dvgo_relu_bit(acc2[r]) << r;
         mask2 |= (unsigned long long)bits << (16 * t2);
-        if (!(experiment & 512)) x3_store_tile(stage, acc2, H2 + tile * 32 * WIDTH + 32 * t2, WIDTH, lane, rows_valid);
+        if constexpr (REC) x3_store_tile_rec(acc2, H2 + tile * 32 * WIDTH, WIDTH, t2, lane, full, valid);
+        else if (!(experiment & 512)) x3_store_tile(stage, acc2, H2 + tile * 32 * WIDTH + 32 * t2, WIDTH, lane, rows_valid);
       }
 #pragma unroll
       for (int c = 0; c < 3; ++c) {
@@ -246,10 +268,12 @@
   float w3p[3][2][T * 16];
 };
 
-template <int WIDTH>
+template <int WIDTH, bool REC>
 struct X3BwdLds : X3BwdImg<WIDTH> {
   float stage[X3_BWD_WAVES][X3_STAGE_ROWS * X3_STAGE_STRIDE];
 };
+template <int WIDTH>
+struct X3BwdLds<WIDTH, true> : X3BwdImg<WIDTH> {};
 
 template <int WIDTH>
 __device__ __forceinline__ void
@@ -297,7 +321,7 @@
   x3_prep_bwd_body<WIDTH>(Lp, W1, W2, W3, D_in, blockIdx.x * blockDim.x + threadIdx.x, gridDim.x * blockDim.x);
 }
 
-template <int WIDTH, bool DIFFUSE>
+template <int WIDTH, bool DIFFUSE, bool REC>
 __global__ void __launch_bounds__(X3_BWD_THREADS)
 shade_bwd_x3_kernel(const float* __restrict__ g_rgb, const float* __restrict__ rgb,
                     const unsigned long long* __restrict__ masks, int64_t M_cap, const int64_t* __restrict__ m_dev,
@@ -305,11 +329,12 @@
                     int n_view, float* __restrict__ g_feat, float* __restrict__ G1, float* __restrict__ gz_out) {
   const int64_t M = m_dev ? (*m_dev < M_cap ? *m_dev : M_cap) : M_cap;
   constexpr int T = WIDTH / 32;
-  __shared__ __attribute__((aligned(16))) X3BwdLds<WIDTH> L;
+  __shared__ __attribute__((aligned(16))) X3BwdLds<WIDTH, REC> L;
   x3_copy_image<X3BwdImg<WIDTH>>(&L, image);
   __syncthreads();
   const int lane = threadIdx.x & 63, h = lane >> 5;
-  float* stage = L.stage[threadIdx.x >> 6];
+  float* stage = nullptr;
+  if constexpr (!REC) stage = L.stage[threadIdx.x >> 6];
   const int64_t n_tiles = (M + 31) / 32;
   const int64_t gw = (int64_t)blockIdx.x * (blockDim.x >> 6) + (threadIdx.x >> 6);
   const int64_t nw = (int64_t)gridDim.x * (blockDim.x >> 6);
@@ -329,6 +354,7 @@
     const int64_t row = tile * 32 + (lane & 31);
     const bool valid = row < M;
     const int rows_valid = (int)(M - tile * 32 < 32 ? M - tile * 32 : 32);
+    const bool full = __builtin_amdgcn_readfirstlane(rows_valid) == 32;
     float gz[3];
 #pragma unroll
     for (int c = 0; c < 3; ++c) gz[c] = valid ? g_n[c] * o_n[c] * (1.0f - o_n[c]) : 0.0f;
@@ -378,7 +404,8 @@
         acc[4 * q + 2] = (mb & 4u) ? acc[4 * q + 2] : 0.0f;
         acc[4 * q + 3] = (mb & 8u) ? acc[4 * q + 3] : 0.0f;
       }
-      x3_store_tile(stage, acc, G1 + tile * 32 * WIDTH + 32 * tin, WIDTH, lane, rows_valid);
+      if constexpr (REC) x3_store_tile_rec(acc, G1 + tile * 32 * WIDTH, WIDTH, tin, lane, full, valid);
+      else x3_store_tile(stage, acc, G1 + tile * 32 * WIDTH + 32 * tin, WIDTH, lane, rows_valid);
 #pragma unroll
       for (int s2 = 0; s2 < 2; ++s2) {
         float v[8];
@@ -1109,11 +1136,12 @@
 int dvgo_shade_fwd_x3(const float* feat, int C, const float* emb, int E, const int64_t* ray_id, int64_t M, const int64_t* m_dev,
                       const float* W1, const float* b1, const float* W2, const float* b2, const float* W3,
                       const float* b3, int width, int d_in, int diffuse, float* rgb, float* H1, float* H2,
-                      uint64_t* masks, void* scratch, void* scratch_bwd, int experiment, void* stream) {
+                      uint64_t* masks, void* scratch, void* scratch_bwd, int experiment, int record, void* stream) {
   if (M < 0 || C <= 0 || E < 0) return DVGO_EINVAL;
   if (M == 0) return 0;
   if (!feat || !emb || !ray_id || !W1 || !b1 || !W2 || !b2 || !W3 || !b3 || !rgb || !scratch) return DVGO_EINVAL;
   if ((H1 == nullptr) != (H2 == nullptr) || (H1 == nullptr) != (masks == nullptr)) return DVGO_EINVAL;
+  if (record && !H1) return DVGO_EINVAL;
   const int c_view0 = diffuse ? 3 : 0;
   const int n_view = C - c_view0;
   if (n_view < 0 || d_in != n_view + E) return DVGO_EINVAL;
@@ -1125,8 +1153,12 @@
 #define DVGO_SHADE_X3(W, KS, DIFF)                                                                                       \
   do {                                                                                                                   \
     x3_prep_fwd_kernel<W, KS><<<scratch_bwd ? 64 : 32, 256, 0, s>>>((X3Img<W, KS>*)scratch, (X3BwdImg<W>*)scratch_bwd, W1, b1, W2, b2, W3, b3, d_in); \
-    shade_fwd_x3_kernel<W, KS, DIFF><<<blocks, X3_THREADS, 0, s>>>(feat, C, c_view0, n_view, emb, E, ray_id, M, m_dev, scratch, rgb, \
-                                                                    H1, H2, (unsigned long long*)masks, experiment);     \
+    if (record)                                                                                                          \
+      shade_fwd_x3_kernel<W, KS, DIFF, true><<<blocks, X3_THREADS, 0, s>>>(feat, C, c_view0, n_view, emb, E, ray_id, M, m_dev, scratch, \
+                                                                           rgb, H1, H2, (unsigned long long*)masks, experiment); \
+    else                                                                                                                 \
+      shade_fwd_x3_kernel<W, KS, DIFF, false><<<blocks, X3_THREADS, 0, s>>>(feat, C, c_view0, n_view, emb, E, ray_id, M, m_dev, scratch, \
+                                                                            rgb, H1, H2, (unsigned long long*)masks, experiment); \
   } while (0)
   if (width == 128) {
     if (diffuse) DVGO_SHADE_X3(128, 3, true); else DVGO_SHADE_X3(128, 3, false);
@@ -1141,7 +1173,7 @@
 
 int dvgo_shade_bwd_x3(const float* g_rgb, const float* rgb, const uint64_t* masks, int64_t M, const int64_t* m_dev,
                       const float* W1, const float* W2, const float* W3, int width, int d_in, int C, int diffuse,
-                      float* g_feat, float* G1, float* gz, void* scratch, int prebuilt, void* stream) {
+                      float* g_feat, float* G1, float* gz, void* scratch, int prebuilt, int record, void* stream) {
   if (M < 0 || C <= 0) return DVGO_EINVAL;
   if (M == 0) return 0;
   if (!g_rgb || !rgb || !masks || !W1 || !W2 || !W3 || !g_feat || !G1 || !gz || !scratch) return DVGO_EINVAL;
@@ -1155,8 +1187,12 @@
 #define DVGO_SHADE_BWD_X3(W, DIFF)                                                                                        \
   do {                                                                                                                    \
     if (!prebuilt) x3_prep_bwd_kernel<W><<<32, 256, 0, s>>>((X3BwdImg<W>*)scratch, W1, W2, W3, d_in);                   \
-    shade_bwd_x3_kernel<W, DIFF><<<blocks, X3_BWD_THREADS, 0, s>>>(g_rgb, rgb, (const unsigned long long*)masks, M, m_dev, scratch, C, \
-                                                                c_view0, n_view, g_feat, G1, gz);                         \
+    if (record)                                                                                                           \
+      shade_bwd_x3_kernel<W, DIFF, true><<<blocks, X3_BWD_THREADS, 0, s>>>(g_rgb, rgb, (const unsigned long long*)masks, M, m_dev, scratch, \
+                                                                           C, c_view0, n_view, g_feat, G1, gz);          \
+    else                                                                                                                  \
+      shade_bwd_x3_kernel<W, DIFF, false><<<blocks, X3_BWD_THREADS, 0, s>>>(g_rgb, rgb, (const unsigned long long*)masks, M, m_dev, scratch, \
+                                                                            C, c_view0, n_view, g_feat, G1, gz);         \
   } while (0)
   if (width == 128) { if (diffuse) DVGO_SHADE_BWD_X3(128, true); else DVGO_SHADE_BWD_X3(128, false); }
   else              { if (diffuse) DVGO_SHADE_BWD_X3(64, true); else DVGO_SHADE_BWD_X3(64, false); }
diff --git a/directvoxgo_amd/shade.py b/directvoxgo_amd/shade.py
--- a/directvoxgo_amd/shade.py
+++ b/directvoxgo_amd/shade.py
@@ -84,6 +84,16 @@
     return gW1, gb1, gW2, gb2, gW3, gb3
 
 
+def record_floats(M_cap, width):
+    return 3 * ((M_cap + 31) // 32) * 32 * width
+
+
+def unpack_activation_record(rec, M, width):
+    tiles = rec.view(3, -1, width // 8, 16, 8)
+    rows = tiles.permute(0, 1, 3, 2, 4).reshape(3, -1, width)
+    return rows[0, :M].clone(), rows[1, :M].clone(), rows[2, :M].clone()
+
+
 def _weight_grads(params, wgrad, device, k, n, g_first=None):
     grads = [g_first] + [None] * (n - 1)
     if defer_wgrad._active is not None:
@@ -102,18 +112,29 @@
         feat, emb = feat.contiguous(), emb.contiguous()
         train = bool(train) and any(ctx.needs_input_grad)
         rgb = torch.empty((M, 3), dtype=torch.float32, device=feat.device)
-        H1 = torch.empty((M, width), dtype=torch.float32, device=feat.device) if train else None
-        H2 = torch.empty((M, width), dtype=torch.float32, device=feat.device) if train else None
         masks = torch.empty((M, 4), dtype=torch.int64, device=feat.device) if train else None
         scratch = _scratch(width, feat.device)
-        scratch_bwd = _scratch(width, feat.device) if (train and (L.lib().dvgo_shade_variant(-1) & 2)) else None
-        with L.device_of(feat):
-            L.call('dvgo_shade_fwd', ptr(feat), _int(C), ptr(emb), _int(E), ptr(ray_id), _i64(M), ptr(m_dev), ptr(W1.contiguous()),
-                   ptr(b1.contiguous()), ptr(W2.contiguous()), ptr(b2.contiguous()), ptr(W3.contiguous()),
-                   ptr(b3.contiguous()), _int(width), _int(d_in), _int(1 if diffuse else 0), ptr(rgb), ptr(H1), ptr(H2),
-                   ptr(masks), ptr(scratch), ptr(scratch_bwd), stream_of(feat))
-        ctx.scratch_bwd = scratch_bwd if (train and (L.lib().dvgo_shade_variant(-1) & 1)) else None
+        variant = L.lib().dvgo_shade_variant(-1)
+        scratch_bwd = _scratch(width, feat.device) if (train and (variant & 2)) else None
+
+        def fwd(H1, H2):
+            with L.device_of(feat):
+                L.call('dvgo_shade_fwd', ptr(feat), _int(C), ptr(emb), _int(E), ptr(ray_id), _i64(M), ptr(m_dev), ptr(W1.contiguous()),
+                       ptr(b1.contiguous()), ptr(W2.contiguous()), ptr(b2.contiguous()), ptr(W3.contiguous()),
+                       ptr(b3.contiguous()), _int(width), _int(d_in), _int(1 if diffuse else 0), ptr(rgb), ptr(H1), ptr(H2),
+                       ptr(masks), ptr(scratch), ptr(scratch_bwd), stream_of(feat))
+
+        record = bool(train and M > 0 and (variant & 128) and (variant & 127) == 67 and scratch is not None)
+        if record:
+            H1, H2 = torch.empty(record_floats(M, width), dtype=torch.float32, device=feat.device), None
+            fwd(H1, None)
+        else:
+            H1 = torch.empty((M, width), dtype=torch.float32, device=feat.device) if train else None
+            H2 = torch.empty((M, width), dtype=torch.float32, device=feat.device) if train else None
+            fwd(H1, H2)
+        ctx.scratch_bwd = scratch_bwd if (train and (variant & 1)) else None
         if train:
+            ctx.record = record
             ctx.save_for_backward(feat, emb, ray_id, W1, W2, W3, rgb, H1, H2, masks)
             ctx.diffuse = diffuse
             ctx.m_dev = m_dev
@@ -128,8 +149,9 @@
         diffuse, m_dev = ctx.diffuse, ctx.m_dev
         M, C = feat.shape
         width, d_in = W1.shape
+        record = ctx.record
         g_feat = torch.empty_like(feat)
-        G1 = torch.empty_like(H1)
+        G1 = H1 if record else torch.empty_like(H1)
         gz = torch.empty_like(rgb)
         prebuilt = ctx.scratch_bwd is not None and W1._version == ctx.w_versions[0] and W2._version == ctx.w_versions[1] \
             and W3._version == ctx.w_versions[2]
@@ -138,7 +160,7 @@
         with L.device_of(feat):
             L.call('dvgo_shade_bwd', ptr(g_rgb.contiguous()), ptr(rgb), ptr(masks), _i64(M), ptr(m_dev), ptr(W1.contiguous()),
                    ptr(W2.contiguous()), ptr(W3.contiguous()), _int(width), _int(d_in), _int(C), _int(1 if diffuse else 0),
-                   ptr(g_feat), ptr(G1), ptr(gz), ptr(scratch), _int(1 if prebuilt else 0), stream_of(feat))
+                   ptr(g_feat), ptr(G1), ptr(gz), ptr(scratch), _int((1 if prebuilt else 0) | (2 if record else 0)), stream_of(feat))
 
         def wgrad():
             n_parts = max(1, min(N_PARTS, (M + 255) // 256))
```

Result: faster. 3.198 million, median of 6 (+1.2%).
